# BesenbacherLab/kmerPaPa

Hardware: NVIDIA B200
Metric: pattern-scores/sec (higher is better)
Workload: dtype f64

## Files before the change

### kmerpapa_b200/csrc/kp_api.cu

```cuda
#include <cuda_runtime.h>
#include <math.h>
#include <stdio.h>
#include <stdlib.h>
#include <string.h>

#include <algorithm>
#include <string>
#include <vector>

#include "../../include/kmerpapa_b200.h"
#include "kp_kernels.cuh"
#include "kp_fiber.cuh"
#include "kp_plan.h"
#include "kp_shard_owners.h"

namespace {

thread_local std::string g_err;

int fail(const std::string &msg)
{
    g_err = msg;
    return KP_ERR;
}

int fail_capacity(const std::string &msg)
{
    g_err = msg;
    return KP_ERR_CAPACITY;
}

#define KP_CUDA(call)                                                                         \
    do {                                                                                      \
        cudaError_t e_ = (call);                                                              \
        if (e_ != cudaSuccess)                                                                \
            return fail(std::string(#call) + ": " + cudaGetErrorString(e_) + " (" + __FILE__ + ":" + \
                        std::to_string(__LINE__) + ")");                                      \
    } while (0)

}

#ifndef KP_PF_TOP
#define KP_PF_TOP 0
#endif
#ifndef KP_EVICT_TOP
#define KP_EVICT_TOP 0
#endif

struct kp_plan {
    KpHostPlan host;
    int device = 0;
    int sm_count = 0;
    KpTables *d_tab = nullptr;
    uint8_t *d_rowtab = nullptr;
    uint32_t *d_tiles = nullptr;
    uint8_t *d_genmask = nullptr;
    int *d_err = nullptr;
    uint32_t *d_counters = nullptr;
    uint8_t *d_tile_wave = nullptr;
    uint8_t *d_tile_done = nullptr;
    unsigned char *d_scratch = nullptr;
    size_t scratch_cap = 0;
    uint64_t launches = 0;
    int nwarps[2] = {0, 0};
    size_t smem_optin = 0;
    bool coop_launch = false;
    KpFiberTables *d_ftab = nullptr;
    uint8_t *d_fiberblob = nullptr;
    uint32_t *d_fibers = nullptr;
    size_t fiber_smem[2] = {0, 0};
    int fiber_dbg = 0;
    bool use_fiber = false;
    int pf_dist = KP_PF_DIST;
    int evict_top = KP_EVICT_TOP;
    bool coop_tail = true;
    int pf_bulk = 0;
    int pf_top = KP_PF_TOP;
    bool one_launch = false;
};

#define KP_RP_NN 232
#ifndef KP_FIBER_DEFAULT
#define KP_FIBER_DEFAULT false
#endif

template <bool WIDE>
static const void *dp_kernel_for_radix(int r0, int rp)
{
    switch (r0) {
    case 1: return (const void *)kp_dp_rows_kernel<1, WIDE, 0, 0>;
    case 3: return (const void *)kp_dp_rows_kernel<3, WIDE, 0, 0>;
    case 7: return (const void *)kp_dp_rows_kernel<7, WIDE, 0, 0>;
    default:
        return rp == KP_RP_NN ? (const void *)kp_dp_rows_kernel<15, WIDE, KP_RP_NN, 0>
                              : (const void *)kp_dp_rows_kernel<15, WIDE, 0, 0>;
    }
}

template <int R0, int RP, int SHARD>
static void launch_dp_r0(bool wide, int grid, int threads, size_t smem, cudaStream_t st, const KpDpParams &prm)
{
    if (wide) kp_dp_rows_kernel<R0, true, RP, SHARD><<<grid, threads, smem, st>>>(prm);
    else kp_dp_rows_kernel<R0, false, RP, SHARD><<<grid, threads, smem, st>>>(prm);
}

template <bool WIDE, int SHARD>
static const void *dp_kernel_sharded(int rp)
{
    return rp == KP_RP_NN ? (const void *)kp_dp_rows_kernel<15, WIDE, KP_RP_NN, SHARD>
                          : (const void *)kp_dp_rows_kernel<15, WIDE, 0, SHARD>;
}

static KpView single_view(const kp_plan *p, const float *best, const uint16_t *flags);

static float tree_sum(const unsigned long long *keys, const float *vals, size_t lo, size_t hi, int depth)
{
    if (hi - lo == 1) return vals[lo];
    const unsigned long long bit = 1ULL << (63 - depth);
    size_t a = lo, b = hi;
    while (a < b) {
        size_t mid = (a + b) / 2;
        if (keys[mid] & bit) b = mid; else a = mid + 1;
    }
    if (a == lo || a == hi) return tree_sum(keys, vals, lo, hi, depth + 1);
    volatile float l = tree_sum(keys, vals, lo, a, depth + 1), r = tree_sum(keys, vals, a, hi, depth + 1);
    volatile float sum = l + r;
    return sum;
}

static KpView single_view(const kp_plan *p, const float *best, const uint16_t *flags)
{
    KpView v;
    memset(&v, 0, sizeof v);
    v.best[0] = best;
    v.flags[0] = flags;
    v.hw_top = (uint32_t)p->host.t.ntiles;
    return v;
}

extern "C" {

const char *kp_last_error(void) { return g_err.c_str(); }
int kp_version(void) { return 100; }

static const void *dp_kernel_ptr(int r0, int rp, bool wide)
{
    return wide ? dp_kernel_for_radix<true>(r0, rp) : dp_kernel_for_radix<false>(r0, rp);
}

static int plan_create(const char *gen_pat, int device, bool lattice, kp_plan **out);

int kp_plan_create(const char *gen_pat, int device, kp_plan **out) { return plan_create(gen_pat, device, true, out); }

int kp_plan_create_lite(const char *gen_pat, int device, kp_plan **out) { return plan_create(gen_pat, device, false, out); }

static int plan_create(const char *gen_pat, int device, bool lattice, kp_plan **out)
{
    if (!gen_pat || !out) return fail("kp_plan_create: null argument");
    int ndev = 0;
    cudaError_t e = cudaGetDeviceCount(&ndev);
    if (e != cudaSuccess || ndev == 0)
        return fail(std::string("kp_plan_create: no CUDA device (") + cudaGetErrorString(e) + "); there is no CPU path");
    if (device < 0 || device >= ndev) return fail("kp_plan_create: bad device ordinal");
    KP_CUDA(cudaSetDevice(device));
    kp_plan *p = new kp_plan();
    std::string err;
    if (kp_build_host_plan(gen_pat, p->host, err, lattice)) { delete p; return fail("kp_plan_create: " + err); }
    p->device = device;
    cudaDeviceProp prop;
    KP_CUDA(cudaGetDeviceProperties(&prop, device));
    p->sm_count = prop.multiProcessorCount;
    const KpTables &t = p->host.t;
    KP_CUDA(cudaMalloc(&p->d_tab, sizeof(KpTables)));
    KP_CUDA(cudaMemcpy(p->d_tab, &t, sizeof(KpTables), cudaMemcpyHostToDevice));
    KP_CUDA(cudaMalloc(&p->d_rowtab, p->host.rowtab.size()));
    KP_CUDA(cudaMemcpy(p->d_rowtab, p->host.rowtab.data(), p->host.rowtab.size(), cudaMemcpyHostToDevice));
    KP_CUDA(cudaMalloc(&p->d_tiles, sizeof(uint32_t) * (p->host.tile_order.size() + 1)));
    KP_CUDA(cudaMemcpy(p->d_tiles, p->host.tile_order.data(), sizeof(uint32_t) * p->host.tile_order.size(), cudaMemcpyHostToDevice));
    KP_CUDA(cudaMalloc(&p->d_genmask, KP_MAXK));
    KP_CUDA(cudaMemcpy(p->d_genmask, p->host.gen_mask, KP_MAXK, cudaMemcpyHostToDevice));
    KP_CUDA(cudaMalloc(&p->d_err, sizeof(int)));
    KP_CUDA(cudaMemset(p->d_err, 0, sizeof(int)));
    KP_CUDA(cudaMalloc(&p->d_counters, sizeof(uint32_t) * 128));
    if (t.r0 == 15 && t.nhigh > 0 && lattice) {
        std::vector<uint8_t> tw(p->host.tile_order.size());
        for (size_t l = 0; l + 1 < p->host.hl_off.size(); l++)
            for (uint64_t i = p->host.hl_off[l]; i < p->host.hl_off[l + 1]; i++) tw[i] = (uint8_t)l;
        KP_CUDA(cudaMalloc(&p->d_tile_wave, tw.size()));
        KP_CUDA(cudaMemcpy(p->d_tile_wave, tw.data(), tw.size(), cudaMemcpyHostToDevice));
        KP_CUDA(cudaMalloc(&p->d_tile_done, tw.size()));
    }
    p->smem_optin = prop.sharedMemPerBlockOptin;
    if (p->host.ft.ok) {
        const KpFiberTables &f = p->host.ft;
        KP_CUDA(cudaMalloc(&p->d_ftab, sizeof(KpFiberTables)));
        KP_CUDA(cudaMemcpy(p->d_ftab, &f, sizeof(KpFiberTables), cudaMemcpyHostToDevice));
        KP_CUDA(cudaMalloc(&p->d_fiberblob, p->host.fibertab.size()));
        KP_CUDA(cudaMemcpy(p->d_fiberblob, p->host.fibertab.data(), p->host.fibertab.size(), cudaMemcpyHostToDevice));
        KP_CUDA(cudaMalloc(&p->d_fibers, sizeof(uint32_t) * (p->host.fiber_order.size() + 1)));
        KP_CUDA(cudaMemcpy(p->d_fibers, p->host.fiber_order.data(), sizeof(uint32_t) * p->host.fiber_order.size(), cudaMemcpyHostToDevice));
        for (int wide = 0; wide < 2; wide++) {
            const size_t need = kp_fiber_smem(f.ft_bytes, f.maxhs, t.tile_kmers, wide != 0).total;
            p->fiber_smem[wide] = need <= p->smem_optin ? need : 0;
        }
        KP_CUDA(cudaFuncSetAttribute((const void *)kp_dp_fiber_kernel<false>, cudaFuncAttributeMaxDynamicSharedMemorySize, (int)prop.sharedMemPerBlockOptin));
        KP_CUDA(cudaFuncSetAttribute((const void *)kp_dp_fiber_kernel<true>, cudaFuncAttributeMaxDynamicSharedMemorySize, (int)prop.sharedMemPerBlockOptin));
        p->use_fiber = KP_FIBER_DEFAULT;
        if (const char *e = getenv("KP_DP_KERNEL")) p->use_fiber = strcmp(e, "fiber") == 0;
        if (const char *e = getenv("KP_FIBER_DBG")) p->fiber_dbg = atoi(e);
    }
    p->coop_launch = prop.cooperativeLaunch != 0 && !getenv("KP_NO_COOP_BACKTRACK");
    if (const char *e = getenv("KP_PF_DIST")) p->pf_dist = atoi(e);
    if (const char *e = getenv("KP_EVICT_TOP")) p->evict_top = atoi(e);
    if (const char *e = getenv("KP_PF_TOP")) p->pf_top = atoi(e);
    if (const char *e = getenv("KP_PF_BULK")) p->pf_bulk = atoi(e);
    if (getenv("KP_NO_COOP_TAIL")) p->coop_tail = false;
    if (const char *e = getenv("KP_ONE_LAUNCH")) p->one_launch = e[0] == '1';
    for (int wide = 0; wide < 2; wide++) {
        size_t fixed = 2048 + t.rt_bytes, per_warp = t.warp_smem_bytes[wide];
        int nw = fixed < p->smem_optin ? (int)((p->smem_optin - fixed) / per_warp) : 0;
        if (nw > KP_MAX_WARPS) nw = KP_MAX_WARPS;
        p->nwarps[wide] = nw;
        KP_CUDA(cudaFuncSetAttribute(dp_kernel_ptr(t.r0, t.rp, wide), cudaFuncAttributeMaxDynamicSharedMemorySize,
                                     (int)prop.sharedMemPerBlockOptin));
        if (t.r0 == 15)
            KP_CUDA(cudaFuncSetAttribute(wide ? dp_kernel_sharded<true, 3>(t.rp) : dp_kernel_sharded<false, 3>(t.rp),
                                         cudaFuncAttributeMaxDynamicSharedMemorySize, (int)prop.sharedMemPerBlockOptin));
    }
    *out = p;
    return 0;
}

int kp_plan_destroy(kp_plan *p)
{
    if (!p) return 0;
    cudaSetDevice(p->device);
    cudaFree(p->d_tab);
    cudaFree(p->d_rowtab);
    cudaFree(p->d_tiles);
    cudaFree(p->d_genmask);
    cudaFree(p->d_err);
    cudaFree(p->d_counters);
    cudaFree(p->d_tile_wave);
    cudaFree(p->d_tile_done);
    cudaFree(p->d_ftab);
    cudaFree(p->d_fiberblob);
    cudaFree(p->d_fibers);
    cudaFree(p->d_scratch);
    delete p;
    return 0;
}

uint64_t kp_backtrack_ws_bytes(uint64_t cap) { return (3 * cap) * sizeof(KpBtNode) + cap * (8 + 8 + 4) + 80 * 8 + 64; }

int kp_plan_get_info(const kp_plan *p, kp_plan_info *o)
{
    if (!p || !o) return fail("kp_plan_get_info: null argument");
    const KpTables &t = p->host.t;
    memset(o, 0, sizeof *o);
    o->npat = p->host.npat;
    o->nkmer = p->host.nkmer;
    o->ntiles = t.ntiles;
    o->table_elems = (uint64_t)t.ntiles * t.tile_stride;
    o->kept_elems = (uint64_t)t.ntiles * (uint64_t)t.rp;
    o->expanded_elems = (uint64_t)t.ntiles * t.tile_kmers;
    o->backtrack_ws_bytes = kp_backtrack_ws_bytes(65536);
    o->k = (uint32_t)p->host.k;
    o->nlevels = t.total_level + 1;
    o->tile_cells = t.tile_cells;
    o->tile_stride = t.tile_stride;
    o->tile_kmers = t.tile_kmers;
    o->low_positions = (uint32_t)t.nlow;
    o->register_radix = (uint32_t)t.r0;
    o->rows = (uint32_t)t.nrows;
    o->rounds = (uint32_t)t.nrounds;
    o->warps_per_cta = (uint32_t)p->nwarps[0];
    o->high_levels = (uint32_t)(p->host.hl_off.size() - 1);
    o->sm_count = (uint32_t)p->sm_count;
    return 0;
}

uint64_t kp_plan_launch_count(const kp_plan *p) { return p ? p->launches : 0; }

const char *kp_dp_kernel_name(const kp_plan *p)
{
    return p && p->use_fiber && p->fiber_smem[0] ? "kp_dp_fiber_kernel" : "kp_dp_rows_kernel";
}

int kp_pattern_offset(const kp_plan *p, uint64_t patnum, uint64_t *table_elem, uint64_t *kept_elem, uint32_t *kept_bit)
{
    if (p && !p->host.lattice) return fail("kp_pattern_offset: this plan was created without the tile lattice (kp_plan_create_lite)");
    if (!p) return fail("kp_pattern_offset: null plan");
    if (patnum >= p->host.npat) return fail("kp_pattern_offset: pattern number out of range");
    uint64_t tile; uint32_t srow, d0;
    kp_locate(p->host, patnum, &tile, &srow, &d0);
    const KpTables &t = p->host.t;
    if (table_elem) *table_elem = tile * t.tile_stride + ((uint64_t)(d0 >> 2) * t.rp + srow) * 4 + (d0 & 3);
    if (kept_elem) *kept_elem = tile * (uint64_t)t.rp + srow;
    if (kept_bit) *kept_bit = d0;
    return 0;
}

static int scratch_reserve(kp_plan *p, size_t bytes, cudaStream_t st)
{
    if (bytes <= p->scratch_cap) return 0;
    KP_CUDA(cudaStreamSynchronize(st));
    if (p->d_scratch) KP_CUDA(cudaFree(p->d_scratch));
    p->d_scratch = nullptr;
    p->scratch_cap = 0;
    size_t cap = bytes + bytes / 2 + 4096;
    KP_CUDA(cudaMalloc(&p->d_scratch, cap));
    p->scratch_cap = cap;
    return 0;
}

static int grid_for(uint64_t n, int threads, int sm_count)
{
    uint64_t b = (n + threads - 1) / threads;
    uint64_t cap = (uint64_t)sm_count * 16;
    if (b > cap) b = cap;
    if (b < 1) b = 1;
    return (int)b;
}

int kp_pack_counts(kp_plan *p, const uint64_t *h_codes, const int64_t *h_pos, const int64_t *h_neg, uint64_t n,
                   int64_t *d_kmerM, int64_t *d_kmerU, void *stream)
{
    if (!p) return fail("kp_pack_counts: null plan");
    if (p->host.k > 16) return fail("kp_pack_counts: packed codes hold at most 16 positions");
    cudaStream_t st = (cudaStream_t)stream;
    KP_CUDA(cudaSetDevice(p->device));
    KP_CUDA(cudaMemsetAsync(d_kmerM, 0, p->host.nkmer * 8, st));
    KP_CUDA(cudaMemsetAsync(d_kmerU, 0, p->host.nkmer * 8, st));
    if (n == 0) return 0;
    if (scratch_reserve(p, n * 24, st)) return 1;
    unsigned long long *d_codes = (unsigned long long *)p->d_scratch;
    long long *d_pos = (long long *)(d_codes + n), *d_neg = d_pos + n;
    KP_CUDA(cudaMemcpyAsync(d_codes, h_codes, n * 8, cudaMemcpyHostToDevice, st));
    KP_CUDA(cudaMemcpyAsync(d_pos, h_pos, n * 8, cudaMemcpyHostToDevice, st));
    KP_CUDA(cudaMemcpyAsync(d_neg, h_neg, n * 8, cudaMemcpyHostToDevice, st));
    KP_CUDA(cudaMemsetAsync(p->d_err, 0, sizeof(int), st));
    kp_pack_kernel<<<grid_for(n, 256, p->sm_count), 256, 0, st>>>(p->d_tab, p->d_genmask, p->host.k, d_codes, d_pos, d_neg, n,
                                                                  (long long *)d_kmerM, (long long *)d_kmerU, p->d_err);
    p->launches++;
    KP_CUDA(cudaGetLastError());
    int herr = 0;
    KP_CUDA(cudaMemcpyAsync(&herr, p->d_err, sizeof(int), cudaMemcpyDeviceToHost, st));
    KP_CUDA(cudaStreamSynchronize(st));
    if (herr) return fail("kp_pack_counts: a k-mer code is not one-hot or lies outside the general pattern");
    return 0;
}

int kp_expand_counts(kp_plan *p, const int64_t *d_kmerM, const int64_t *d_kmerU, int64_t *d_expM, int64_t *d_expU,
                     void *stream)
{
    if (!p) return fail("kp_expand_counts: null plan");
    if (!p->host.lattice) return fail("kp_expand_counts: this plan was created without the tile lattice (kp_plan_create_lite)");
    cudaStream_t st = (cudaStream_t)stream;
    KP_CUDA(cudaSetDevice(p->device));
    const KpTables &t = p->host.t;
    kp_expand_base_kernel<<<grid_for(p->host.nkmer, 256, p->sm_count), 256, 0, st>>>(
        p->d_tab, p->host.nkmer, (const long long *)d_kmerM, (const long long *)d_kmerU, (long long *)d_expM, (long long *)d_expU);
    p->launches++;
    for (int hi = 0; hi < t.nhigh; hi++) {
        uint64_t total = t.tile_kmers;
        for (int h = 0; h < t.nhigh; h++) {
            const int f = t.highpos[h];
            total *= h < hi ? (uint64_t)t.radix[f] : (h == hi ? (uint64_t)(t.radix[f] - t.nbase[f]) : (uint64_t)t.nbase[f]);
        }
        if (total == 0) continue;
        kp_expand_pass_kernel<<<grid_for(total, 256, p->sm_count), 256, 0, st>>>(p->d_tab, hi, total, (long long *)d_expM,
                                                                                 (long long *)d_expU);
        p->launches++;
    }
    KP_CUDA(cudaGetLastError());
    return 0;
}

static int launch_dp(kp_plan *p, bool wide, KpDpParams prm, cudaStream_t st)
{
    if (!p->host.lattice) return fail("this plan was created without the tile lattice (kp_plan_create_lite): no DP");
    int nw = p->nwarps[wide];
    if (nw < 1) return fail("DP kernel does not fit in shared memory for this tile shape");
    size_t nhl = p->host.hl_off.size() - 1;
    const KpTables &t = p->host.t;
    if (nhl > 64) return fail("too many tile waves");
    KP_CUDA(cudaMemsetAsync(p->d_counters, 0, sizeof(uint32_t) * 128, st));
    if (p->use_fiber && p->fiber_smem[wide]) {
        KpFiberParams fp;
        memset(&fp, 0, sizeof fp);
        fp.tab = p->d_tab; fp.ftab = p->d_ftab; fp.fiberblob = p->d_fiberblob;
        fp.e0 = prm.e0; fp.e1 = prm.e1; fp.s0 = prm.s0; fp.s1 = prm.s1;
        fp.alpha = prm.alpha; fp.beta = prm.beta; fp.penalty = prm.penalty;
        fp.best = prm.best; fp.flags = prm.flags;
        fp.dbg = p->fiber_dbg;
        const size_t nfl = p->host.fl_off.size() - 1;
        for (size_t l = 0; l < nfl; l++) {
            const uint64_t lo = p->host.fl_off[l], hi = p->host.fl_off[l + 1];
            if (hi == lo) continue;
            fp.fiber_list = p->d_fibers + lo;
            fp.nfibers_wave = (uint32_t)(hi - lo);
            fp.counter = p->d_counters + l;
            fp.leaf_wave = (l == 0);
            const int grid = (int)std::min<uint64_t>(hi - lo, (uint64_t)p->sm_count);
            if (wide) kp_dp_fiber_kernel<true><<<grid, KP_FIBER_THREADS, p->fiber_smem[1], st>>>(fp);
            else kp_dp_fiber_kernel<false><<<grid, KP_FIBER_THREADS, p->fiber_smem[0], st>>>(fp);
            p->launches++;
        }
        KP_CUDA(cudaGetLastError());
        return 0;
    }
    if (p->d_tile_done && t.ntiles >= (uint64_t)8 * p->sm_count * nw && p->one_launch) {
        KP_CUDA(cudaMemsetAsync(p->d_tile_done, 0, t.ntiles, st));
        KP_CUDA(cudaMemsetAsync(p->d_err, 0, sizeof(int), st));
        prm.tile_list = p->d_tiles;
        prm.ntiles_wave = (uint32_t)t.ntiles;
        prm.counter = p->d_counters;
        prm.leaf_wave = 0;
        prm.tile_wave = p->d_tile_wave;
        prm.tile_done = p->d_tile_done;
        prm.wave_done = p->d_counters + 64;
        prm.err = p->d_err;
        for (size_t l = 0; l < 64; l++) prm.wave_size[l] = l < nhl ? (uint32_t)(p->host.hl_off[l + 1] - p->host.hl_off[l]) : 0;
        const size_t sm = 2048 + t.rt_bytes + (size_t)nw * t.warp_smem_bytes[wide];
        if (t.rp == KP_RP_NN) launch_dp_r0<15, KP_RP_NN, 3>(wide, p->sm_count, nw * 32, sm, st, prm);
        else launch_dp_r0<15, 0, 3>(wide, p->sm_count, nw * 32, sm, st, prm);
        p->launches++;
        KP_CUDA(cudaGetLastError());
        return 0;
    }
    for (size_t l = 0; l < nhl; l++) {
        uint64_t lo = p->host.hl_off[l], hi = p->host.hl_off[l + 1];
        if (hi == lo) continue;
        prm.tile_list = p->d_tiles + lo;
        prm.ntiles_wave = (uint32_t)(hi - lo);
        prm.counter = p->d_counters + l;
        prm.leaf_wave = (l == 0);
        uint64_t ntile = hi - lo;
        const int nchunk = (t.nrows + 31) / 32;
        if (p->coop_tail && t.r0 == 15 && ntile <= (uint64_t)p->sm_count && nchunk <= KP_MAX_WARPS) {
            const size_t smc = 2048 + t.rt_bytes + (size_t)t.warp_smem_bytes[wide];
            if (t.rp == KP_RP_NN) launch_dp_r0<15, KP_RP_NN, 4>(wide, (int)ntile, nchunk * 32, smc, st, prm);
            else launch_dp_r0<15, 0, 4>(wide, (int)ntile, nchunk * 32, smc, st, prm);
            p->launches++;
            continue;
        }
        int warps = nw;
        if (ntile < (uint64_t)p->sm_count * nw) {
            warps = (int)((ntile + p->sm_count - 1) / p->sm_count);
            if (warps < 1) warps = 1;
        }
        uint64_t grid = (ntile + warps - 1) / warps;
        if (grid > (uint64_t)p->sm_count) grid = p->sm_count;
        size_t sm = 2048 + t.rt_bytes + (size_t)warps * t.warp_smem_bytes[wide];
        switch (t.r0) {
        case 1: launch_dp_r0<1, 0, 0>(wide, (int)grid, warps * 32, sm, st, prm); break;
        case 3: launch_dp_r0<3, 0, 0>(wide, (int)grid, warps * 32, sm, st, prm); break;
        case 7: launch_dp_r0<7, 0, 0>(wide, (int)grid, warps * 32, sm, st, prm); break;
        default:
            if (t.rp == KP_RP_NN) launch_dp_r0<15, KP_RP_NN, 0>(wide, (int)grid, warps * 32, sm, st, prm);
            else launch_dp_r0<15, 0, 0>(wide, (int)grid, warps * 32, sm, st, prm);
            break;
        }
        p->launches++;
    }
    KP_CUDA(cudaGetLastError());
    return 0;
}

static int dp_counts(kp_plan *p, const int64_t *d_expM, const int64_t *d_expU, const int64_t *d_subM, const int64_t *d_subU,
                     uint64_t max_count, double alpha, double beta, double penalty, float *d_best, uint16_t *d_kept, void *stream);

int kp_dp_single(kp_plan *p, const int64_t *d_expM, const int64_t *d_expU, uint64_t max_count, double alpha, double beta,
                 double penalty, float *d_best, uint16_t *d_kept, void *stream)
{
    return dp_counts(p, d_expM, d_expU, nullptr, nullptr, max_count, alpha, beta, penalty, d_best, d_kept, stream);
}

static int dp_counts(kp_plan *p, const int64_t *d_expM, const int64_t *d_expU, const int64_t *d_subM, const int64_t *d_subU,
                     uint64_t max_count, double alpha, double beta, double penalty, float *d_best, uint16_t *d_kept, void *stream)
{
    if (!p) return fail("kp_dp_single: null plan");
    KP_CUDA(cudaSetDevice(p->device));
    bool wide = max_count > 0xFFFFFFFFull;
    KpDpParams prm;
    memset(&prm, 0, sizeof prm);
    prm.tab = p->d_tab;
    prm.rowtab = p->d_rowtab;
    prm.e0 = (const long long *)d_expM;
    prm.e1 = (const long long *)d_expU;
    prm.s0 = (const long long *)d_subM;
    prm.s1 = (const long long *)d_subU;
    prm.alpha = alpha; prm.beta = beta; prm.penalty = penalty;
    prm.best = d_best;
    prm.flags = d_kept;
    prm.pf_dist = p->pf_dist;
    prm.evict_top = p->evict_top < p->host.t.nhigh ? p->evict_top : 0;
    prm.pf_top = p->pf_top;
    prm.pf_bulk = p->pf_bulk;
    return launch_dp(p, wide, prm, (cudaStream_t)stream);
}

static int backtrack_device(kp_plan *p, const KpView &vw, void *d_ws, uint64_t cap, uint64_t root,
                            cudaStream_t st, unsigned long long **sorted_out, unsigned long long **keys_out, float **vals_out,
                            unsigned long long **ctr_out)
{
    KpBtNode *fa = (KpBtNode *)d_ws, *fb = fa + cap, *leaves = fb + cap;
    unsigned long long *sorted = (unsigned long long *)(leaves + cap);
    unsigned long long *keys = sorted + cap;
    unsigned long long *ctr = keys + cap;
    float *vals = (float *)(ctr + 80);
    kp_backtrack_init_kernel<<<1, 128, 0, st>>>(fa, root, ctr);
    const int levels = (int)p->host.t.total_level + 1;
    int grid = (int)((cap + 7) / 8);
    if (grid > p->sm_count * 2) grid = p->sm_count * 2;
    bool fused = false;
    if (p->coop_launch) {
        int nlev = levels < 64 ? levels : 64;
        int cgrid = grid < p->sm_count ? grid : p->sm_count;
        const KpTables *a_tab = p->d_tab;
        const uint8_t *a_row = p->d_rowtab;
        void *args[] = {(void *)&a_tab, (void *)&a_row, (void *)&vw, (void *)&nlev, (void *)&fa, (void *)&fb, (void *)&leaves,
                        (void *)&cap, (void *)&ctr};
        if (cudaLaunchCooperativeKernel((const void *)kp_backtrack_all_kernel, dim3(cgrid), dim3(256), args, 0, st) == cudaSuccess) {
            fused = true;
            p->launches++;
        } else {
            cudaGetLastError();
        }
    }
    for (int d = 0; !fused && d < levels && d < 64; d++) {
        kp_backtrack_level_kernel<<<grid, 256, 0, st>>>(p->d_tab, p->d_rowtab, vw, d, (d & 1) ? fb : fa,
                                                        (d & 1) ? fa : fb, leaves, cap, ctr);
        p->launches++;
    }
    kp_backtrack_sort_kernel<<<p->sm_count, 256, 0, st>>>(leaves, ctr, cap, sorted, keys);
    p->launches += 2;
    KP_CUDA(cudaGetLastError());
    *sorted_out = sorted; *keys_out = keys; *vals_out = vals; *ctr_out = ctr;
    return 0;
}

int kp_backtrack(kp_plan *p, const float *d_best, const uint16_t *d_kept, void *d_ws, uint64_t cap, uint64_t root,
                 uint64_t *h_patnums, uint64_t *n_out, void *stream)
{
    if (!p || !d_ws || !h_patnums || !n_out) return fail("kp_backtrack: null argument");
    if (p->host.t.total_level > 64) return fail("kp_backtrack: more than 64 levels");
    if (root == UINT64_MAX) root = p->host.npat - 1;
    if (root >= p->host.npat) return fail("kp_backtrack: root out of range");
    cudaStream_t st = (cudaStream_t)stream;
    KP_CUDA(cudaSetDevice(p->device));
    unsigned long long *sorted, *keys, *ctr;
    float *vals;
    if (backtrack_device(p, single_view(p, d_best, d_kept), d_ws, cap, root, st, &sorted, &keys, &vals, &ctr)) return 1;
    unsigned long long hc[2] = {0, 0};
    int herr = 0;
    KP_CUDA(cudaMemcpyAsync(hc, ctr, sizeof hc, cudaMemcpyDeviceToHost, st));
    KP_CUDA(cudaMemcpyAsync(&herr, p->d_err, sizeof herr, cudaMemcpyDeviceToHost, st));
    KP_CUDA(cudaStreamSynchronize(st));
    if (herr == 2) return fail("kp_backtrack: the DP gave up waiting for a child tile (internal error)");
    *n_out = hc[0];
    if (hc[1] || hc[0] > cap) return fail_capacity("kp_backtrack: partition larger than the workspace capacity");
    KP_CUDA(cudaMemcpyAsync(h_patnums, sorted, hc[0] * 8, cudaMemcpyDeviceToHost, st));
    KP_CUDA(cudaStreamSynchronize(st));
    return 0;
}

int kp_cv_heldout(kp_plan *p, const float *d_train, const uint16_t *d_kept, const int64_t *d_expMtot, const int64_t *d_expUtot,
                  const int64_t *d_expMtest, const int64_t *d_expUtest, double alpha, double beta_fold, double penalty,
                  uint64_t root, void *d_ws, uint64_t cap, float *h_test, void *stream)
{
    if (!p || !d_ws || !h_test) return fail("kp_cv_heldout: null argument");
    if (root == UINT64_MAX) root = p->host.npat - 1;
    if (root >= p->host.npat) return fail("kp_cv_heldout: root out of range");
    cudaStream_t st = (cudaStream_t)stream;
    KP_CUDA(cudaSetDevice(p->device));
    unsigned long long *sorted, *keys, *ctr;
    float *vals;
    if (backtrack_device(p, single_view(p, d_train, d_kept), d_ws, cap, root, st, &sorted, &keys, &vals, &ctr)) return 1;
    kp_cv_leaf_kernel<<<p->sm_count, 128, 0, st>>>(p->d_tab, p->d_rowtab, (const long long *)d_expMtot, (const long long *)d_expUtot,
                                                   (const long long *)d_expMtest, (const long long *)d_expUtest, alpha, beta_fold,
                                                   penalty, sorted, ctr, cap, vals);
    p->launches++;
    KP_CUDA(cudaGetLastError());
    unsigned long long hc[2] = {0, 0};
    KP_CUDA(cudaMemcpyAsync(hc, ctr, sizeof hc, cudaMemcpyDeviceToHost, st));
    KP_CUDA(cudaStreamSynchronize(st));
    if (hc[1] || hc[0] > cap) return fail_capacity("kp_cv_heldout: partition larger than the workspace capacity");
    if (hc[0] == 0) return fail("kp_cv_heldout: the backtrack produced no leaf (internal error)");
    std::vector<unsigned long long> hk(hc[0]);
    std::vector<float> hv(hc[0]);
    KP_CUDA(cudaMemcpyAsync(hk.data(), keys, hc[0] * 8, cudaMemcpyDeviceToHost, st));
    KP_CUDA(cudaMemcpyAsync(hv.data(), vals, hc[0] * 4, cudaMemcpyDeviceToHost, st));
    KP_CUDA(cudaStreamSynchronize(st));
    *h_test = tree_sum(hk.data(), hv.data(), 0, hc[0], 0);
    return 0;
}

int kp_dp_cv_job(kp_plan *p, const int64_t *d_expMtot, const int64_t *d_expUtot, const int64_t *d_expMtest,
                 const int64_t *d_expUtest, uint64_t max_count, double alpha, double beta_fold, double penalty,
                 float *d_train, uint16_t *d_kept, void *d_ws, uint64_t cap, float *h_top, void *stream)
{
    if (!p || !d_expMtest || !d_expUtest) return fail("kp_dp_cv_job: null argument");
    cudaStream_t st = (cudaStream_t)stream;
    KP_CUDA(cudaSetDevice(p->device));
    const KpTables &t = p->host.t;
    if (dp_counts(p, d_expMtot, d_expUtot, d_expMtest, d_expUtest, max_count, alpha, beta_fold, penalty, d_train, d_kept, stream))
        return 1;
    if (h_top) {
        if (int rc = kp_cv_heldout(p, d_train, d_kept, d_expMtot, d_expUtot, d_expMtest, d_expUtest, alpha, beta_fold, penalty,
                                   UINT64_MAX, d_ws, cap, h_top + 1, stream))
            return rc;
        uint64_t tile; uint32_t srow, d0;
        kp_locate(p->host, p->host.npat - 1, &tile, &srow, &d0);
        size_t top = (size_t)tile * t.tile_stride + ((size_t)(d0 >> 2) * t.rp + srow) * 4 + (d0 & 3);
        KP_CUDA(cudaMemcpyAsync(h_top, d_train + top, sizeof(float), cudaMemcpyDeviceToHost, st));
        KP_CUDA(cudaStreamSynchronize(st));
    }
    return 0;
}

uint64_t kp_cv_stage_bytes(uint64_t cap) { return 32 + cap * 12; }

int kp_cv_job_enqueue(kp_plan *p, const int64_t *d_expMtot, const int64_t *d_expUtot, const int64_t *d_expMtest,
                      const int64_t *d_expUtest, uint64_t max_count, double alpha, double beta_fold, double penalty,
                      float *d_train, uint16_t *d_kept, void *d_ws, uint64_t cap, void *h_stage, void *stream)
{
    if (!p || !d_expMtest || !d_expUtest || !d_ws || !h_stage) return fail("kp_cv_job_enqueue: null argument");
    cudaStream_t st = (cudaStream_t)stream;
    KP_CUDA(cudaSetDevice(p->device));
    const KpTables &t = p->host.t;
    if (dp_counts(p, d_expMtot, d_expUtot, d_expMtest, d_expUtest, max_count, alpha, beta_fold, penalty, d_train, d_kept, stream))
        return 1;
    unsigned long long *sorted, *keys, *ctr;
    float *vals;
    if (backtrack_device(p, single_view(p, d_train, d_kept), d_ws, cap, p->host.npat - 1, st, &sorted, &keys, &vals, &ctr)) return 1;
    kp_cv_leaf_kernel<<<p->sm_count, 128, 0, st>>>(p->d_tab, p->d_rowtab, (const long long *)d_expMtot, (const long long *)d_expUtot,
                                                   (const long long *)d_expMtest, (const long long *)d_expUtest, alpha, beta_fold,
                                                   penalty, sorted, ctr, cap, vals);
    p->launches++;
    KP_CUDA(cudaGetLastError());
    unsigned char *h = (unsigned char *)h_stage;
    uint64_t tile; uint32_t srow, d0;
    kp_locate(p->host, p->host.npat - 1, &tile, &srow, &d0);
    const size_t top = (size_t)tile * t.tile_stride + ((size_t)(d0 >> 2) * t.rp + srow) * 4 + (d0 & 3);
    KP_CUDA(cudaMemcpyAsync(h, ctr, 16, cudaMemcpyDeviceToHost, st));
    KP_CUDA(cudaMemcpyAsync(h + 16, d_train + top, sizeof(float), cudaMemcpyDeviceToHost, st));
    KP_CUDA(cudaMemcpyAsync(h + 32, keys, cap * 8, cudaMemcpyDeviceToHost, st));
    KP_CUDA(cudaMemcpyAsync(h + 32 + cap * 8, vals, cap * 4, cudaMemcpyDeviceToHost, st));
    return 0;
}

int kp_cv_job_finish(const void *h_stage, uint64_t cap, float *h_top)
{
    if (!h_stage || !h_top) return fail("kp_cv_job_finish: null argument");
    const unsigned char *h = (const unsigned char *)h_stage;
    unsigned long long hc[2];
    memcpy(hc, h, 16);
    if (hc[1] || hc[0] > cap) return fail_capacity("kp_cv_job_finish: partition larger than the workspace capacity");
    if (hc[0] == 0) return fail("kp_cv_job_finish: the backtrack produced no leaf (internal error)");
    memcpy(h_top, h + 16, sizeof(float));
    h_top[1] = tree_sum((const unsigned long long *)(h + 32), (const float *)(h + 32 + cap * 8), 0, hc[0], 0);
    return 0;
}

int kp_split_codes(kp_plan *p, const float *d_best, const uint16_t *d_kept, const uint64_t *h_patnums, uint64_t n,
                   uint8_t *h_codes, void *stream)
{
    if (!p) return fail("kp_split_codes: null plan");
    if (n == 0) return 0;
    cudaStream_t st = (cudaStream_t)stream;
    KP_CUDA(cudaSetDevice(p->device));
    if (scratch_reserve(p, n * 9, st)) return 1;
    unsigned long long *d_pat = (unsigned long long *)p->d_scratch;
    uint8_t *d_codes = (uint8_t *)(d_pat + n);
    KP_CUDA(cudaMemcpyAsync(d_pat, h_patnums, n * 8, cudaMemcpyHostToDevice, st));
    kp_split_codes_kernel<<<grid_for(n, 256, p->sm_count), 256, 0, st>>>(p->d_tab, p->d_rowtab, single_view(p, d_best, d_kept), d_pat, n, d_codes);
    p->launches++;
    KP_CUDA(cudaGetLastError());
    KP_CUDA(cudaMemcpyAsync(h_codes, d_codes, n, cudaMemcpyDeviceToHost, st));
    KP_CUDA(cudaStreamSynchronize(st));
    return 0;
}

int kp_gather_table(kp_plan *p, const float *d_table, uint64_t first, uint64_t n, float *h_out, void *stream)
{
    if (!p) return fail("kp_gather_table: null plan");
    if (n == 0) return 0;
    cudaStream_t st = (cudaStream_t)stream;
    KP_CUDA(cudaSetDevice(p->device));
    if (scratch_reserve(p, n * 4, st)) return 1;
    float *d_out = (float *)p->d_scratch;
    kp_gather_kernel<<<grid_for(n, 256, p->sm_count), 256, 0, st>>>(p->d_tab, p->d_rowtab, single_view(p, d_table, nullptr), nullptr, first, n, d_out);
    p->launches++;
    KP_CUDA(cudaGetLastError());
    KP_CUDA(cudaMemcpyAsync(h_out, d_out, n * 4, cudaMemcpyDeviceToHost, st));
    KP_CUDA(cudaStreamSynchronize(st));
    return 0;
}

int kp_gather_kept(kp_plan *p, const uint16_t *d_kept, uint64_t first, uint64_t n, uint8_t *h_out, void *stream)
{
    if (!p) return fail("kp_gather_kept: null plan");
    if (n == 0) return 0;
    cudaStream_t st = (cudaStream_t)stream;
    KP_CUDA(cudaSetDevice(p->device));
    if (scratch_reserve(p, n, st)) return 1;
    uint8_t *d_out = (uint8_t *)p->d_scratch;
    kp_gather_flags_kernel<<<grid_for(n, 256, p->sm_count), 256, 0, st>>>(p->d_tab, p->d_rowtab, single_view(p, nullptr, d_kept), nullptr, first, n, d_out);
    p->launches++;
    KP_CUDA(cudaGetLastError());
    KP_CUDA(cudaMemcpyAsync(h_out, d_out, n, cudaMemcpyDeviceToHost, st));
    KP_CUDA(cudaStreamSynchronize(st));
    return 0;
}

int kp_gather_patterns(kp_plan *p, const float *d_table, const uint16_t *d_kept, const uint64_t *h_patnums, uint64_t n,
                       float *h_best, uint8_t *h_kept, uint8_t *h_codes, void *stream)
{
    if (!p || !h_patnums) return fail("kp_gather_patterns: null argument");
    if (!p->host.lattice) return fail("kp_gather_patterns: this plan was created without the tile lattice (kp_plan_create_lite)");
    if ((h_best || h_codes) && !d_table) return fail("kp_gather_patterns: scores and split codes need the score table");
    if ((h_kept || h_codes) && !d_kept) return fail("kp_gather_patterns: kept flags and split codes need the kept-whole table");
    if (n == 0) return 0;
    cudaStream_t st = (cudaStream_t)stream;
    KP_CUDA(cudaSetDevice(p->device));
    if (scratch_reserve(p, n * 16, st)) return 1;
    unsigned long long *d_pat = (unsigned long long *)p->d_scratch;
    float *d_val = (float *)(d_pat + n);
    uint8_t *d_k = (uint8_t *)(d_val + n), *d_c = d_k + n;
    KP_CUDA(cudaMemcpyAsync(d_pat, h_patnums, n * 8, cudaMemcpyHostToDevice, st));
    const int grid = grid_for(n, 256, p->sm_count);
    const KpView vw = single_view(p, d_table, d_kept);
    if (h_best) { kp_gather_kernel<<<grid, 256, 0, st>>>(p->d_tab, p->d_rowtab, vw, d_pat, 0, n, d_val); p->launches++; }
    if (h_kept) { kp_gather_flags_kernel<<<grid, 256, 0, st>>>(p->d_tab, p->d_rowtab, vw, d_pat, 0, n, d_k); p->launches++; }
    if (h_codes) { kp_split_codes_kernel<<<grid, 256, 0, st>>>(p->d_tab, p->d_rowtab, vw, d_pat, n, d_c); p->launches++; }
    KP_CUDA(cudaGetLastError());
    if (h_best) KP_CUDA(cudaMemcpyAsync(h_best, d_val, n * 4, cudaMemcpyDeviceToHost, st));
    if (h_kept) KP_CUDA(cudaMemcpyAsync(h_kept, d_k, n, cudaMemcpyDeviceToHost, st));
    if (h_codes) KP_CUDA(cudaMemcpyAsync(h_codes, d_c, n, cudaMemcpyDeviceToHost, st));
    KP_CUDA(cudaStreamSynchronize(st));
    return 0;
}

int kp_pattern_counts(kp_plan *p, const int64_t *d_kmerM, const int64_t *d_kmerU, const uint64_t *h_patnums, uint64_t n,
                      int64_t *h_M, int64_t *h_U, void *stream)
{
    if (!p) return fail("kp_pattern_counts: null plan");
    if (n == 0) return 0;
    cudaStream_t st = (cudaStream_t)stream;
    KP_CUDA(cudaSetDevice(p->device));
    if (scratch_reserve(p, n * 24, st)) return 1;
    unsigned long long *d_pat = (unsigned long long *)p->d_scratch;
    long long *d_out = (long long *)(d_pat + n);
    KP_CUDA(cudaMemcpyAsync(d_pat, h_patnums, n * 8, cudaMemcpyHostToDevice, st));
    const int pc_grid = (int)std::min<uint64_t>(n, (uint64_t)p->sm_count * 16);
    kp_pattern_counts_kernel<<<pc_grid, 256, 0, st>>>(p->d_tab, n, (const long long *)d_kmerM, (const long long *)d_kmerU,
                                                      d_pat, d_out, d_out + n);
    p->launches++;
    KP_CUDA(cudaGetLastError());
    KP_CUDA(cudaMemcpyAsync(h_M, d_out, n * 8, cudaMemcpyDeviceToHost, st));
    KP_CUDA(cudaMemcpyAsync(h_U, d_out + n, n * 8, cudaMemcpyDeviceToHost, st));
    KP_CUDA(cudaStreamSynchronize(st));
    return 0;
}

struct PartLayout {
    unsigned long long *pat, *pm, *offs, *bsum;
};

static size_t part_bytes(uint64_t n) { return (3 * n + 1 + 1024) * 8; }

static PartLayout part_layout(const kp_plan *p, uint64_t n)
{
    PartLayout L;
    L.pat = (unsigned long long *)p->d_scratch;
    L.pm = L.pat + n;
    L.offs = L.pm + n;
    L.bsum = L.offs + n + 1;
    return L;
}

static int part_check(const kp_plan *p, const char *what, const uint64_t *h_patnums, uint64_t n)
{
    if (!p) return fail(std::string(what) + ": null plan");
    if (!h_patnums || n == 0) return fail(std::string(what) + ": empty partition");
    if (n >= KP_OWNER_EMPTY) return fail(std::string(what) + ": too many patterns (owners are uint32)");
    for (uint64_t i = 0; i < n; i++)
        if (h_patnums[i] >= p->host.npat) return fail(std::string(what) + ": pattern number out of range");
    return 0;
}

static int part_prepare(kp_plan *p, const uint64_t *h_patnums, uint64_t n, cudaStream_t st, uint64_t *total)
{
    const PartLayout L = part_layout(p, n);
    KP_CUDA(cudaMemcpyAsync(L.pat, h_patnums, n * 8, cudaMemcpyHostToDevice, st));
    const uint64_t nb = std::min<uint64_t>(1024, (n + 255) / 256), per = (n + nb - 1) / nb;
    kp_part_prep_kernel<<<(unsigned)nb, 256, 0, st>>>(p->d_tab, L.pat, n, per, L.pm, L.bsum);
    kp_part_scan_kernel<<<1, 256, 0, st>>>(L.bsum, (unsigned)nb, L.offs, n);
    kp_part_offsets_kernel<<<(unsigned)nb, 256, 0, st>>>(p->d_tab, L.pm, n, per, L.bsum, L.offs);
    p->launches += 3;
    KP_CUDA(cudaGetLastError());
    unsigned long long tot = 0;
    KP_CUDA(cudaMemcpyAsync(&tot, L.offs + n, 8, cudaMemcpyDeviceToHost, st));
    KP_CUDA(cudaStreamSynchronize(st));
    *total = tot;
    return 0;
}

int kp_partition_assign(kp_plan *p, const uint64_t *h_patnums, uint64_t n, uint32_t *d_owner, uint64_t *h_conflict,
                        uint64_t *h_uncovered, void *stream)
{
    if (part_check(p, "kp_partition_assign", h_patnums, n)) return KP_ERR;
    if (!d_owner || !h_conflict || !h_uncovered) return fail("kp_partition_assign: null argument");
    cudaStream_t st = (cudaStream_t)stream;
    KP_CUDA(cudaSetDevice(p->device));
    if (scratch_reserve(p, part_bytes(n) + 16, st)) return KP_ERR;
    const PartLayout L = part_layout(p, n);
    unsigned long long *d_res = L.bsum + 1024;
    uint64_t total = 0;
    if (part_prepare(p, h_patnums, n, st, &total)) return KP_ERR;
    const uint64_t nkmer = p->host.nkmer;
    KP_CUDA(cudaMemsetAsync(d_owner, 0xFF, nkmer * 4, st));
    KP_CUDA(cudaMemsetAsync(d_res, 0xFF, 16, st));
    const int grid = p->sm_count * 8;
    unsigned long long res[2] = {~0ull, ~0ull};
    for (uint64_t lo = 0; lo < total; lo += nkmer) {
        const uint64_t hi = std::min<uint64_t>(total, lo + nkmer);
        kp_part_assign_kernel<<<grid, 256, 0, st>>>(p->d_tab, L.pm, L.offs, n, lo, hi, d_owner, d_res);
        p->launches++;
        KP_CUDA(cudaGetLastError());
        if (hi == total) break;
        KP_CUDA(cudaMemcpyAsync(res, d_res, 8, cudaMemcpyDeviceToHost, st));
        KP_CUDA(cudaStreamSynchronize(st));
        if (res[0] != ~0ull) break;
    }
    KP_CUDA(cudaMemcpyAsync(res, d_res, 8, cudaMemcpyDeviceToHost, st));
    KP_CUDA(cudaStreamSynchronize(st));
    if (res[0] == ~0ull) {
        kp_part_cover_kernel<<<grid_for(nkmer, 256, p->sm_count), 256, 0, st>>>(d_owner, nkmer, d_res);
        p->launches++;
        KP_CUDA(cudaGetLastError());
        KP_CUDA(cudaMemcpyAsync(res, d_res, 16, cudaMemcpyDeviceToHost, st));
        KP_CUDA(cudaStreamSynchronize(st));
    }
    *h_conflict = res[0] == ~0ull ? 0 : res[0] + 1;
    *h_uncovered = res[0] != ~0ull || res[1] == ~0ull ? 0 : res[1] + 1;
    return 0;
}

int kp_partition_score(kp_plan *p, const uint64_t *h_patnums, const double *h_rate, uint64_t n, const int64_t *d_kmerM,
                       const int64_t *d_kmerU, const uint32_t *d_owner, double *d_kmer_rate, int64_t *h_M, int64_t *h_U,
                       double *h_t, void *stream)
{
    if (part_check(p, "kp_partition_score", h_patnums, n)) return KP_ERR;
    if (!h_rate || !d_kmerM || !d_kmerU || !h_M || !h_U || !h_t) return fail("kp_partition_score: null argument");
    if (d_kmer_rate && !d_owner) return fail("kp_partition_score: the per-k-mer rates need the owner table");
    cudaStream_t st = (cudaStream_t)stream;
    KP_CUDA(cudaSetDevice(p->device));
    if (scratch_reserve(p, part_bytes(n) + 4 * n * 8, st)) return KP_ERR;
    const PartLayout L = part_layout(p, n);
    unsigned long long *d_M = (unsigned long long *)((unsigned char *)p->d_scratch + part_bytes(n)), *d_U = d_M + n;
    double *d_rate = (double *)(d_U + n), *d_t = d_rate + n;
    uint64_t total = 0;
    if (part_prepare(p, h_patnums, n, st, &total)) return KP_ERR;
    if (total > p->host.nkmer) return fail("kp_partition_score: the patterns have more members than there are k-mers (they overlap)");
    KP_CUDA(cudaMemcpyAsync(d_rate, h_rate, n * 8, cudaMemcpyHostToDevice, st));
    KP_CUDA(cudaMemsetAsync(d_M, 0, 2 * n * 8, st));
    kp_part_counts_kernel<<<p->sm_count * 8, 256, 0, st>>>(p->d_tab, L.pm, L.offs, n, total, (const long long *)d_kmerM,
                                                           (const long long *)d_kmerU, d_M, d_U);
    kp_part_terms_kernel<<<grid_for(n, 256, p->sm_count), 256, 0, st>>>(d_M, d_U, d_rate, n, d_t);
    p->launches += 2;
    if (d_kmer_rate) {
        kp_part_kmer_rate_kernel<<<grid_for(p->host.nkmer, 256, p->sm_count), 256, 0, st>>>(d_owner, d_rate, n, p->host.nkmer,
                                                                                           d_kmer_rate);
        p->launches++;
    }
    KP_CUDA(cudaGetLastError());
    KP_CUDA(cudaMemcpyAsync(h_M, d_M, n * 8, cudaMemcpyDeviceToHost, st));
    KP_CUDA(cudaMemcpyAsync(h_U, d_U, n * 8, cudaMemcpyDeviceToHost, st));
    KP_CUDA(cudaMemcpyAsync(h_t, d_t, n * 8, cudaMemcpyDeviceToHost, st));
    KP_CUDA(cudaStreamSynchronize(st));
    return 0;
}

int kp_kmer_rates(kp_plan *p, const uint32_t *d_owner, const double *h_rate, uint64_t n, double *d_kmer_rate, void *stream)
{
    if (!p) return fail("kp_kmer_rates: null plan");
    if (!d_owner || !h_rate || !d_kmer_rate || n == 0) return fail("kp_kmer_rates: null argument");
    cudaStream_t st = (cudaStream_t)stream;
    KP_CUDA(cudaSetDevice(p->device));
    if (scratch_reserve(p, n * 8, st)) return KP_ERR;
    double *d_rate = (double *)p->d_scratch;
    KP_CUDA(cudaMemcpyAsync(d_rate, h_rate, n * 8, cudaMemcpyHostToDevice, st));
    kp_part_kmer_rate_kernel<<<grid_for(p->host.nkmer, 256, p->sm_count), 256, 0, st>>>(d_owner, d_rate, n, p->host.nkmer,
                                                                                       d_kmer_rate);
    p->launches++;
    KP_CUDA(cudaGetLastError());
    KP_CUDA(cudaStreamSynchronize(st));
    return 0;
}

int kp_seq_scan(kp_plan *p, const uint8_t *d_seq, uint64_t seq_base, uint64_t seq_len, uint64_t rec_len, uint64_t pos0,
                uint64_t pos1, int both, const double *d_kmer_rate, const uint32_t *d_tasks, uint64_t ntask, double *d_sum,
                int64_t *d_n, float *d_track, const uint32_t *d_count_mask, int64_t *d_counts, void *stream)
{
    if (!p) return fail("kp_seq_scan: null plan");
    const int k = p->host.k, c = k / 2;
    if (!d_seq || !d_kmer_rate || !d_sum || !d_n) return fail("kp_seq_scan: null argument");
    if ((uintptr_t)d_seq & 15) return fail("kp_seq_scan: the sequence buffer must be 16-byte aligned");
    if (both && k % 2 == 0) return fail("kp_seq_scan: both strands need an odd k");
    if (pos0 % KP_SEQ_PIECE || pos0 > pos1 || pos1 > rec_len) return fail("kp_seq_scan: bad position range");
    const uint64_t need_lo = pos0 >= (uint64_t)c ? pos0 - c : 0, need_hi = std::min<uint64_t>(rec_len, pos1 + (k - 1 - c));
    if (pos1 > pos0 && (seq_base > need_lo || seq_base + seq_len < need_hi || seq_base + seq_len > rec_len))
        return fail("kp_seq_scan: the sequence bytes do not cover the windows of the positions");
    if (d_tasks && (d_track || d_counts)) return fail("kp_seq_scan: tracks and counts come from the whole-piece pass");
    if (pos1 == pos0 || (d_tasks && ntask == 0)) return 0;
    if (!d_tasks && (pos1 - pos0 + KP_SEQ_PIECE - 1) / KP_SEQ_PIECE > 0x7FFFFFFFull) return fail("kp_seq_scan: too many pieces");
    if (d_tasks && ntask > 0x7FFFFFFFull) return fail("kp_seq_scan: too many tasks");
    cudaStream_t st = (cudaStream_t)stream;
    KP_CUDA(cudaSetDevice(p->device));
    KpSeqScan a;
    a.seq = d_seq;
    a.seq_base = seq_base;
    a.seq_len = seq_len;
    a.rec_len = rec_len;
    a.pos0 = pos0;
    a.pos1 = pos1;
    a.kmer_rate = d_kmer_rate;
    a.tasks = d_tasks;
    a.sum = d_sum;
    a.n = (unsigned long long *)d_n;
    a.track = d_track;
    a.count_mask = d_count_mask;
    a.counts = (unsigned long long *)d_counts;
    a.k = k;
    a.c = c;
    const unsigned grid = (unsigned)(d_tasks ? ntask : (pos1 - pos0 + KP_SEQ_PIECE - 1) / KP_SEQ_PIECE);
    if (both) kp_seq_scan_kernel<true><<<grid, KP_SEQ_THREADS, 0, st>>>(p->d_tab, p->d_genmask, a);
    else kp_seq_scan_kernel<false><<<grid, KP_SEQ_THREADS, 0, st>>>(p->d_tab, p->d_genmask, a);
    p->launches++;
    KP_CUDA(cudaGetLastError());
    return 0;
}

int kp_region_sums(kp_plan *p, const double *d_piece_sum, const int64_t *d_piece_n, const double *d_task_sum,
                   const int64_t *d_task_n, const int64_t *d_regions, uint64_t n, double *d_sum, int64_t *d_n, void *stream)
{
// ... 659 lines not shown
```

### kmerpapa_b200/csrc/kp_fiber.cuh

```cuda
#pragma once
#include "kp_kernels.cuh"

#define KP_FIBER_THREADS 512
#define KP_FIBER_CELLS (KP_FIBER_DIGITS * KP_FIBER_ROWS)

struct KpFiberParams {
    const KpTables *tab;
    const KpFiberTables *ftab;
    const uint8_t *fiberblob;
    const uint32_t *fiber_list;
    uint32_t nfibers_wave;
    uint32_t *counter;
    int leaf_wave;
    const long long *e0, *e1;
    const long long *s0, *s1;
    double alpha, beta, penalty;
    float *best;
    uint16_t *flags;
    int dbg;
};

struct KpFiberSmem {
    uint32_t logtab, blob, bc, hs, misc, fsplit, flags, planes, total;
};

__host__ __device__ inline KpFiberSmem kp_fiber_smem(uint32_t ft_bytes, uint32_t maxhs, uint32_t tile_kmers, bool wide)
{
    KpFiberSmem m;
    uint32_t o = 0;
    m.logtab = o; o += 2048;
    m.blob = o; o += (ft_bytes + 15u) & ~15u;
    m.bc = o; o += KP_FIBER_DIGITS * tile_kmers * 2u * (wide ? 8u : 4u);
    m.hs = o; o += ((maxhs * 8u) + 15u) & ~15u;
    m.misc = o; o += 256;
    m.fsplit = o; o += 256;
    m.flags = o; o += (KP_FIBER_CELLS * 2u + 15u) & ~15u;
    m.planes = o; o += KP_FIBER_CELLS * 60u;
    m.total = o;
    return m;
}

struct KpFiberS {
    float4 *P0, *P1, *P2;
    float *Q0, *Q1, *Q2;
    __device__ __forceinline__ void load(int idx, float *v) const
    {
        const float4 a = P0[idx], b = P1[idx], c = P2[idx];
        v[0] = a.x; v[1] = a.y; v[2] = a.z; v[3] = a.w;
        v[4] = b.x; v[5] = b.y; v[6] = b.z; v[7] = b.w;
        v[8] = c.x; v[9] = c.y; v[10] = c.z; v[11] = c.w;
        v[12] = Q0[idx]; v[13] = Q1[idx]; v[14] = Q2[idx];
    }
    __device__ __forceinline__ void store(int idx, const float *v) const
    {
        P0[idx] = make_float4(v[0], v[1], v[2], v[3]);
        P1[idx] = make_float4(v[4], v[5], v[6], v[7]);
        P2[idx] = make_float4(v[8], v[9], v[10], v[11]);
        Q0[idx] = v[12]; Q1[idx] = v[13]; Q2[idx] = v[14];
    }
};

__device__ __forceinline__ void kp_fiber_split1(const KpFiberS &S, int ia, int ib, float *v)
{
    float xa[16], xb[16];
    S.load(ia, xa);
    S.load(ib, xb);
#pragma unroll
    for (int c = 0; c < 14; c += 2) {
        const float2 s = __fadd2_rn(make_float2(xa[c], xa[c + 1]), make_float2(xb[c], xb[c + 1]));
        v[c] = fminf(v[c], s.x);
        v[c + 1] = fminf(v[c + 1], s.y);
    }
    v[14] = fminf(v[14], __fadd_rn(xa[14], xb[14]));
}

__device__ __forceinline__ void kp_fiber_split2(const KpFiberS &S, int ia, int ib, int ic, int ie, float *v)
{
    float xa[16], xb[16], xc[16], xe[16];
    S.load(ia, xa);
    S.load(ib, xb);
    S.load(ic, xc);
    S.load(ie, xe);
#pragma unroll
    for (int c = 0; c < 14; c += 2) {
        const float2 s1 = __fadd2_rn(make_float2(xa[c], xa[c + 1]), make_float2(xb[c], xb[c + 1]));
        const float2 s2 = __fadd2_rn(make_float2(xc[c], xc[c + 1]), make_float2(xe[c], xe[c + 1]));
        v[c] = kp_min3(v[c], s1.x, s2.x);
        v[c + 1] = kp_min3(v[c + 1], s1.y, s2.y);
    }
    v[14] = kp_min3(v[14], __fadd_rn(xa[14], xb[14]), __fadd_rn(xc[14], xe[14]));
}

__device__ __forceinline__ float4 kp_min4(float4 m, float4 a, float4 b)
{
    const float2 lo = __fadd2_rn(make_float2(a.x, a.y), make_float2(b.x, b.y));
    const float2 hi = __fadd2_rn(make_float2(a.z, a.w), make_float2(b.z, b.w));
    return make_float4(fminf(m.x, lo.x), fminf(m.y, lo.y), fminf(m.z, hi.x), fminf(m.w, hi.y));
}

template <bool WIDE>
__global__ void __launch_bounds__(KP_FIBER_THREADS, 1) kp_dp_fiber_kernel(const KpFiberParams p)
{
    typedef typename KpCnt<WIDE>::type C;
    constexpr int R0 = 15, NB = 4, NT = KP_FIBER_THREADS, NR = KP_FIBER_ROWS, RP = 232;
    constexpr int TILE4 = 4 * RP;
    constexpr int NJ = KP_FIBER_DIGITS * TILE4;

    extern __shared__ __align__(16) unsigned char smem[];
    const KpTables &tb = *p.tab;
    const KpFiberTables &ft = *p.ftab;
    const int tid = threadIdx.x;
    const uint32_t tk = tb.tile_kmers;
    const KpFiberSmem sm = kp_fiber_smem(ft.ft_bytes, ft.maxhs, tk, WIDE);

    double2 *logtab = (double2 *)(smem + sm.logtab);
    unsigned char *blob = smem + sm.blob;
    C *bc = (C *)(smem + sm.bc);
    uint32_t *hs1 = (uint32_t *)(smem + sm.hs), *hs2 = hs1 + ft.maxhs;
    int *misc = (int *)(smem + sm.misc);
    uint8_t *fsplit = smem + sm.fsplit;
    uint16_t *sflags = (uint16_t *)(smem + sm.flags);
    KpFiberS S;
    S.P0 = (float4 *)(smem + sm.planes);
    S.P1 = S.P0 + KP_FIBER_CELLS;
    S.P2 = S.P1 + KP_FIBER_CELLS;
    S.Q0 = (float *)(S.P2 + KP_FIBER_CELLS);
    S.Q1 = S.Q0 + KP_FIBER_CELLS;
    S.Q2 = S.Q1 + KP_FIBER_CELLS;

    for (int i = tid; i < 128; i += NT) logtab[i] = make_double2(kpc_logTab[2 * i], kpc_logTab[2 * i + 1]);
    for (uint32_t i = tid; i < ft.ft_bytes / 4; i += NT) ((uint32_t *)blob)[i] = ((const uint32_t *)p.fiberblob)[i];
    if (tid < KP_FIBER_DIGITS) {
        const int e = ft.fe, d = tid;
        const uint32_t m = tb.digit_mask[e][d];
        const int ns = tb.ms_n[m];
        for (int j = 0; j < ns; j++) {
            fsplit[(d * 8 + j) * 2 + 0] = tb.mask_digit[e][tb.ms_c1[m][j]];
            fsplit[(d * 8 + j) * 2 + 1] = tb.mask_digit[e][tb.ms_c2[m][j]];
        }
        fsplit[240 + d] = (uint8_t)ns;
    }
    __syncthreads();
    const uint8_t *frow_of_srow = blob + ft.ft_frow_of_srow;
    const uint16_t *xs_off = (const uint16_t *)(blob + ft.ft_xs_off);
    const uint16_t *xs = (const uint16_t *)(blob + ft.ft_xs);
    const uint16_t *bs_off = (const uint16_t *)(blob + ft.ft_bs_off);
    const uint8_t *bs = blob + ft.ft_bs;
    uint32_t lvl_start[KP_FIBER_ROW_LEVELS + 1];
#pragma unroll
    for (int l = 0; l <= KP_FIBER_ROW_LEVELS; l++) lvl_start[l] = ft.lvl_start[l];

    const double alpha = p.alpha, beta = p.beta, penalty = p.penalty;
    const KpFilterK fk = kp_filter_consts(alpha, beta, penalty);
    const float INF = __int_as_float(0x7f800000);
    const uint32_t hwf = ft.hw;
    const int nhigh = tb.nhigh, fhi = ft.fhi;
    const float4 *tb4 = (const float4 *)p.best;

    for (;;) {
        __syncthreads();
        if (tid == 0) misc[0] = (int)atomicAdd(p.counter, 1u);
        __syncthreads();
        const uint32_t it = (uint32_t)misc[0];
        if (it >= p.nfibers_wave) break;
        const uint32_t base = p.fiber_list[it];
        if (tid < 32) {
            int ns = 0, d = 0, e = 0;
            uint32_t m = 0, hw = 1;
            if (tid < nhigh && tid != fhi) {
                e = tb.highpos[tid];
                hw = tb.highw[e];
                d = (int)((base / hw) % tb.radix[e]);
                m = tb.digit_mask[e][d];
                ns = tb.ms_n[m];
            }
            int off = ns;
#pragma unroll
            for (int o = 1; o < 32; o <<= 1) {
                int x = __shfl_up_sync(0xffffffffu, off, o);
                if (tid >= o) off += x;
            }
            const int total = __shfl_sync(0xffffffffu, off, 31);
            off -= ns;
            for (int j = 0; j < ns; j++) {
                const int c1 = tb.mask_digit[e][tb.ms_c1[m][j]], c2 = tb.mask_digit[e][tb.ms_c2[m][j]];
                hs1[off + j] = base - (uint32_t)(d - c1) * hw;
                hs2[off + j] = base - (uint32_t)(d - c2) * hw;
            }
            if (tid == 0) misc[1] = total;
        }
        for (uint32_t i = tid; i < KP_FIBER_DIGITS * tk; i += NT) {
            const uint32_t x = i / tk, kl = i - x * tk;
            const size_t g = (size_t)(base + x * hwf) * tk + kl;
            bc[i * 2 + 0] = (C)(p.s0 ? p.e0[g] - p.s0[g] : p.e0[g]);
            bc[i * 2 + 1] = (C)(p.s1 ? p.e1[g] - p.s1[g] : p.e1[g]);
        }
        __syncthreads();
        const int nhs = misc[1];

        for (int j0 = tid; j0 < ((p.dbg & 1) ? 0 : NJ); j0 += 2 * NT) {
            const int j1 = j0 + NT;
            const int x0 = j0 / TILE4, r0 = j0 - x0 * TILE4;
            const int x1 = j1 / TILE4, r1 = j1 - x1 * TILE4;
            const int g0 = r0 / RP, srow0 = r0 - g0 * RP;
            const int g1 = r1 / RP, srow1 = r1 - g1 * RP;
            const bool ok0 = srow0 < NR, ok1 = j1 < NJ && srow1 < NR;
            const size_t o0 = (size_t)x0 * hwf * TILE4 + r0, o1 = (size_t)x1 * hwf * TILE4 + r1;
            float4 acc0 = make_float4(INF, INF, INF, INF), acc1 = acc0;
            for (int s0 = 0; s0 < nhs; s0 += 4) {
                float4 a0[4], b0[4], a1[4], b1[4];
#pragma unroll
                for (int q = 0; q < 4; q++) {
                    a0[q] = b0[q] = a1[q] = b1[q] = make_float4(INF, INF, INF, INF);
                    if (s0 + q < nhs) {
                        const float4 *c1 = tb4 + (size_t)hs1[s0 + q] * TILE4, *c2 = tb4 + (size_t)hs2[s0 + q] * TILE4;
                        if (ok0) { a0[q] = __ldg(c1 + o0); b0[q] = __ldg(c2 + o0); }
                        if (ok1) { a1[q] = __ldg(c1 + o1); b1[q] = __ldg(c2 + o1); }
                    }
                }
#pragma unroll
                for (int q = 0; q < 4; q++) {
                    acc0 = kp_min4(acc0, a0[q], b0[q]);
                    acc1 = kp_min4(acc1, a1[q], b1[q]);
                }
            }
            if (ok0) {
                const int idx = x0 * NR + frow_of_srow[srow0];
                if (g0 == 0) S.P0[idx] = acc0;
                else if (g0 == 1) S.P1[idx] = acc0;
                else if (g0 == 2) S.P2[idx] = acc0;
                else { S.Q0[idx] = acc0.x; S.Q1[idx] = acc0.y; S.Q2[idx] = acc0.z; }
            }
            if (ok1) {
                const int idx = x1 * NR + frow_of_srow[srow1];
                if (g1 == 0) S.P0[idx] = acc1;
                else if (g1 == 1) S.P1[idx] = acc1;
                else if (g1 == 2) S.P2[idx] = acc1;
                else { S.Q0[idx] = acc1.x; S.Q1[idx] = acc1.y; S.Q2[idx] = acc1.z; }
            }
        }
        __syncthreads();

        for (int L = 0; L <= ((p.dbg & 2) ? -1 : 3 + KP_FIBER_ROW_LEVELS - 1); L++) {
            int gstart[5];
            gstart[0] = 0;
#pragma unroll
            for (int lx = 0; lx < 4; lx++) {
                const int lr = L - lx;
                const int nx = lx == 0 ? 4 : (lx == 1 ? 6 : (lx == 2 ? 4 : 1));
                int nr = 0;
#pragma unroll
                for (int l = 0; l < KP_FIBER_ROW_LEVELS; l++)
                    if (l == lr) nr = (int)(lvl_start[l + 1] - lvl_start[l]);
                gstart[lx + 1] = gstart[lx] + nx * nr;
            }
            for (int k = tid; k < gstart[4]; k += NT) {
                const int lx = k < gstart[1] ? 0 : (k < gstart[2] ? 1 : (k < gstart[3] ? 2 : 3));
                const int lr = L - lx;
                const int xbase = lx == 0 ? 0 : (lx == 1 ? 4 : (lx == 2 ? 10 : 14));
                int rstart = 0, nr = 1;
#pragma unroll
                for (int l = 0; l < KP_FIBER_ROW_LEVELS; l++)
                    if (l == lr) { rstart = (int)lvl_start[l]; nr = (int)(lvl_start[l + 1] - lvl_start[l]); }
                const int kk = k - gstart[lx];
                const int xi = kk / nr;
                const int x = xbase + xi, frow = rstart + (kk - xi * nr);
                const int idx = x * NR + frow;

                float v[16];
                S.load(idx, v);
                v[15] = INF;
                {
                    const int nfs = fsplit[240 + x];
                    const uint8_t *fs = fsplit + x * 16;
                    int j = 0;
                    for (; j + 2 <= nfs; j += 2)
                        kp_fiber_split2(S, fs[2 * j] * NR + frow, fs[2 * j + 1] * NR + frow, fs[2 * j + 2] * NR + frow,
                                        fs[2 * j + 3] * NR + frow, v);
                    if (j < nfs) kp_fiber_split1(S, fs[2 * j] * NR + frow, fs[2 * j + 1] * NR + frow, v);
                }
                {
                    int i = xs_off[frow];
                    const int iend = xs_off[frow + 1];
                    const int xb = x * NR;
                    for (; i + 2 <= iend; i += 2) {
                        const uint32_t pr = xs[i], pq = xs[i + 1];
                        kp_fiber_split2(S, xb + (int)(pr & 0xFFu), xb + (int)(pr >> 8), xb + (int)(pq & 0xFFu), xb + (int)(pq >> 8), v);
                    }
                    if (i < iend) {
                        const uint32_t pr = xs[i];
                        kp_fiber_split1(S, xb + (int)(pr & 0xFFu), xb + (int)(pr >> 8), v);
                    }
                }
                C m[NB], u[NB];
#pragma unroll
                for (int b = 0; b < NB; b++) { m[b] = 0; u[b] = 0; }
                {
                    const C *bcx = bc + (size_t)x * tk * 2;
                    for (int i = bs_off[frow]; i < bs_off[frow + 1]; i++) {
                        const C *q = bcx + (size_t)bs[i] * NB * 2;
                        if (!WIDE) {
#pragma unroll
                            for (int b = 0; b < NB; b += 2) {
                                const uint4 y = *(const uint4 *)(q + b * 2);
                                m[b] += y.x; u[b] += y.y; m[b + 1] += y.z; u[b + 1] += y.w;
                            }
                        } else {
#pragma unroll
                            for (int b = 0; b < NB; b++) { m[b] += q[b * 2 + 0]; u[b] += q[b * 2 + 1]; }
                        }
                    }
                }
                const bool leafrow = p.leaf_wave != 0 && lx == 0 && lr == 0;
                uint32_t need = 0;
                {
                    float mf[NB], uf[NB];
#pragma unroll
                    for (int b = 0; b < NB; b++) { mf[b] = (float)m[b]; uf[b] = (float)u[b]; }
#pragma unroll
                    for (int h = 0; h < (R0 + 1) / 2; h++) {
                        float2 Mf = make_float2(0.f, 0.f), Uf = make_float2(0.f, 0.f);
#pragma unroll
                        for (int b = 0; b < NB; b++) {
                            if ((kp_bm_c<R0>(2 * h) >> b) & 1) { Mf.x += mf[b]; Uf.x += uf[b]; }
                            if (2 * h + 1 < R0 && ((kp_bm_c<R0>(2 * h + 1) >> b) & 1)) { Mf.y += mf[b]; Uf.y += uf[b]; }
                        }
                        const float2 lb = kp_score_lower_bound2(Mf, Uf, fk);
                        if (!(lb.x > v[2 * h])) need |= 1u << (2 * h);
                        if (2 * h + 1 < R0 && !(lb.y > v[2 * h + 1])) need |= 1u << (2 * h + 1);
                    }
                    if (leafrow) need |= (1u << NB) - 1u;
                }
                float sfx[16];
#pragma unroll
                for (int c = 0; c < 16; c++) sfx[c] = 0.f;
                uint32_t rupm = 0;
                if (need) {
                    const KpLogK K = kp_logk_load();
                    uint32_t todo = need;
                    while (todo) {
                        const int d = __ffs(todo) - 1;
                        todo &= todo - 1;
                        const unsigned bm = kp_bm<R0>(d);
                        C M_ = 0, U_ = 0;
#pragma unroll
                        for (int b = 0; b < NB; b++)
                            if ((bm >> b) & 1u) { M_ += m[b]; U_ += u[b]; }
                        float sf;
                        bool ru;
                        const bool leafcell = leafrow && d < NB;
                        if (leafcell || !kp_self_score_fast<C>(M_, U_, alpha, beta, penalty, logtab, K, sf, ru)) {
                            const double s_ = leafcell ? kp_leaf_score_nl(M_, U_, alpha, beta, penalty, logtab)
                                                       : kp_self_score_exact_nl<C>(M_, U_, alpha, beta, penalty, logtab);
                            sf = __double2float_rn(s_);
                            ru = (double)sf > s_;
                        }
                        if (ru) rupm |= 1u << d;
#pragma unroll
                        for (int c = 0; c < R0; c++)
                            if (c == d) sfx[c] = sf;
                    }
                }
                uint32_t flag = 0;
#define KP_FIN(D)                                                                                     \
    if ((need >> (D)) & 1u) {                                                                         \
        const float sf_ = sfx[D];                                                                     \
        if (sf_ < v[D] || (sf_ == v[D] && ((rupm >> (D)) & 1u))) { v[D] = sf_; flag |= 1u << (D); }   \
    }
#define KP_SP(D, A, B) v[D] = fminf(v[D], __fadd_rn(v[A], v[B]));
#define KP_SP2(D, A, B, A2, B2) v[D] = kp_min3(v[D], __fadd_rn(v[A], v[B]), __fadd_rn(v[A2], v[B2]));
                KP_FIN(0) KP_FIN(1) KP_FIN(2) KP_FIN(3)
                KP_SP(4, 0, 2) KP_FIN(4)
                KP_SP(5, 1, 3) KP_FIN(5)
                KP_SP(6, 2, 1) KP_FIN(6)
                KP_SP(7, 0, 3) KP_FIN(7)
                KP_SP(8, 2, 3) KP_FIN(8)
                KP_SP(9, 0, 1) KP_FIN(9)
                KP_SP2(10, 1, 8, 2, 5) KP_SP(10, 3, 6) KP_FIN(10)
                KP_SP2(11, 0, 8, 2, 7) KP_SP(11, 3, 4) KP_FIN(11)
                KP_SP2(12, 0, 5, 1, 7) KP_SP(12, 3, 9) KP_FIN(12)
                KP_SP2(13, 0, 6, 1, 4) KP_SP(13, 2, 9) KP_FIN(13)
                KP_SP2(14, 6, 7, 8, 9) KP_SP2(14, 4, 5, 0, 10)
                KP_SP2(14, 1, 11, 2, 12) KP_SP(14, 3, 13) KP_FIN(14)
#undef KP_FIN
#undef KP_SP
#undef KP_SP2
                S.store(idx, v);
                sflags[idx] = (uint16_t)flag;
            }
            __syncthreads();
        }

        for (int j = tid; j < NJ; j += NT) {
            const int x = j / TILE4, r = j - x * TILE4;
            const int g = r / RP, srow = r - g * RP;
            if (srow >= NR) continue;
            const int idx = x * NR + frow_of_srow[srow];
            float4 o;
            if (g == 0) o = S.P0[idx];
            else if (g == 1) o = S.P1[idx];
            else if (g == 2) o = S.P2[idx];
            else o = make_float4(S.Q0[idx], S.Q1[idx], S.Q2[idx], 0.f);
            __stcs((float4 *)p.best + (size_t)(base + x * hwf) * TILE4 + r, o);
        }
        for (int j = tid; j < KP_FIBER_DIGITS * RP; j += NT) {
            const int x = j / RP, srow = j - x * RP;
            if (srow < NR) p.flags[(size_t)(base + x * hwf) * RP + srow] = sflags[x * NR + frow_of_srow[srow]];
        }
    }
}
```

### kmerpapa_b200/csrc/kp_kernels.cuh

```cuda
#pragma once
#include <cuda_runtime.h>
#include <stdint.h>

#include "kp_math.cuh"
#include "kp_tables.h"

#ifndef KP_MAX_WARPS
#define KP_MAX_WARPS 12
#endif
#define KP_DP_BOUNDS __launch_bounds__(KP_MAX_WARPS * 32, 1)
#ifndef KP_PIPE_DEPTH
#define KP_PIPE_DEPTH 2
#endif
#ifndef KP_EXPERIMENTS
#define KP_EXPERIMENTS 0
#endif
#ifndef KP_PF_DIST
#define KP_PF_DIST 2
#endif

template <bool WIDE> struct KpCnt { typedef unsigned int type; };
template <> struct KpCnt<true> { typedef unsigned long long type; };

__device__ __forceinline__ double kp_cnt2d(unsigned int x) { return __uint2double_rn(x); }
__device__ __forceinline__ double kp_cnt2d(unsigned long long x) { return __ull2double_rn(x); }

template <typename C>
__device__ __forceinline__ double kp_self_score_t(C M, C U, double alpha, double beta, double penalty,
                                                  const double2 *tab, const KpLogK &K, double &logp, double &log1mp)
{
    double Md = kp_cnt2d(M), Ud = kp_cnt2d(U);
    double p = __ddiv_rn(KP_ADD(Md, alpha), KP_ADD(KP_ADD(kp_cnt2d((C)(M + U)), alpha), beta));
    double q = KP_SUB(1.0, p);
    int phi = __double2hiint(p), qhi = __double2hiint(q), qlo = __double2loint(q);
    if (kp_log_is_plain(phi) && !kp_log_is_near1(phi)) logp = kp_log_main(phi, __double2loint(p), tab, K);
    else logp = kp_log_slow(p, tab);
    if (kp_log_is_near1(qhi) && !(qhi == 0x3ff00000 && qlo == 0)) log1mp = kp_log_near1(q, K);
    else log1mp = kp_log_slow(q, tab);
    double s1 = KP_ADD(penalty, KP_MUL(KP_MUL(-2.0, Md), logp));
    double s = M > 0 ? s1 : penalty;
    double s2 = KP_ADD(s, KP_MUL(KP_MUL(-2.0, Ud), log1mp));
    return U > 0 ? s2 : s;
}

template <typename C>
__device__ __noinline__ double kp_self_score_exact_nl(C M, C U, double alpha, double beta, double penalty, const double2 *tab)
{
    const KpLogK K = kp_logk_load();
    double lp, l1;
    return kp_self_score_t<C>(M, U, alpha, beta, penalty, tab, K, lp, l1);
}

#ifndef KP_FAST_INLINE
#define KP_FAST_INLINE __forceinline__
#endif
template <typename C>
__device__ KP_FAST_INLINE bool kp_self_score_fast(C M, C U, double alpha, double beta, double penalty, const double2 *tab,
                                                   const KpLogK &K, float &sf, bool &rup, double *st = nullptr)
{
    const double Md = kp_cnt2d(M), Ud = kp_cnt2d(U), Sd = kp_cnt2d((C)(M + U));
    const double num = KP_ADD(Md, alpha), den = KP_ADD(KP_ADD(Sd, alpha), beta);
    double r;
    asm("rcp.approx.ftz.f64 %0, %1;" : "=d"(r) : "d"(den));
    double e = KP_FMA(-den, r, 1.0);
    r = KP_FMA(r, e, r);
    e = KP_FMA(-den, r, 1.0);
    r = KP_FMA(r, e, r);
    const double p = KP_MUL(num, r);
    const int phi = __double2hiint(p), dhi = __double2hiint(den);
    bool ok = (unsigned)(phi - 0x01700000) < (unsigned)(0x3fb00000 - 0x01700000) &&
              (unsigned)(dhi - 0x20b00000) < (unsigned)(0x5f300000 - 0x20b00000) && penalty >= 0.0;
    const double *A = kpc_logA;
    const unsigned thi = (unsigned)phi - 0x3fe60000u;
    const int i = (int)((thi >> 13) & 127u);
    const int k = (int)thi >> 20;
    const double z = __hiloint2double(phi - (int)(thi & 0xfff00000u), __double2loint(p));
    const double2 t = tab[i];
    const double kd = (double)k;
    const double rr = KP_FMA(z, t.x, -1.0);
    const double r2 = KP_MUL(rr, rr);
    const double w = KP_FMA(kd, KP_LOG_LN2HI, t.y);
    double q1 = KP_FMA(rr, A[4], K.a3);
    const double q5 = KP_FMA(rr, A[2], K.a1);
    q1 = KP_FMA(q1, r2, q5);
    double lo = KP_FMA(kd, KP_LOG_LN2LO, rr);
    lo = KP_FMA(r2, A[0], lo);
    lo = KP_FMA(KP_MUL(rr, r2), q1, lo);
    const double logp = KP_ADD(w, lo);
    const double *B = kpc_logB;
    const double x = KP_SUB(KP_SUB(1.0, p), 1.0);
    const double x2 = KP_MUL(x, x);
    double y;
    if (phi < 0x3f700000) {
        y = KP_FMA(x, B[4], B[3]);
        y = KP_FMA(y, x, B[2]);
        y = KP_FMA(y, x, K.b1);
        y = KP_FMA(y, x, -0.5);
    } else {
        y = KP_FMA(x, B[10], B[9]);
        y = KP_FMA(y, x, B[8]);
        y = KP_FMA(y, x, K.b7);
        y = KP_FMA(y, x, B[6]);
        y = KP_FMA(y, x, B[5]);
        y = KP_FMA(y, x, K.b4);
        y = KP_FMA(y, x, B[3]);
        y = KP_FMA(y, x, B[2]);
        y = KP_FMA(y, x, K.b1);
        y = KP_FMA(y, x, -0.5);
    }
    const double logq = KP_FMA(x2, y, x);
    const double t1 = KP_MUL(KP_MUL(-2.0, Md), logp), t2 = KP_MUL(KP_MUL(-2.0, Ud), logq);
    double sa = M > 0 ? KP_ADD(penalty, t1) : penalty;
    sa = U > 0 ? KP_ADD(sa, t2) : sa;
    const double eps = KP_FMA(sa, 0x1p-46, KP_MUL(Sd, 0x1p-49));
    const double slo = KP_SUB(sa, eps), shi = KP_ADD(sa, eps);
    const float flo = __double2float_rn(slo), fhi = __double2float_rn(shi);
    const double fd = (double)flo;
    sf = flo;
    rup = fd > shi;
    if (st) *st = sa;
    ok = ok && flo == fhi && (fd > shi || fd < slo) && sa < 0x1p120;
    return ok;
}

template <typename C>
__device__ __forceinline__ double kp_test_ll_t(C Mt, C Ut, double logp, double log1mp)
{
    double t1 = KP_ADD(0.0, KP_MUL(KP_MUL(-2.0, kp_cnt2d(Mt)), logp));
    double t = Mt > 0 ? t1 : 0.0;
    double t2 = KP_ADD(t, KP_MUL(KP_MUL(-2.0, kp_cnt2d(Ut)), log1mp));
    return Ut > 0 ? t2 : t;
}

template <int BM, int NB, typename C>
__device__ __forceinline__ C kp_sum_bases(const C *x)
{
    C s = 0;
#pragma unroll
    for (int b = 0; b < NB; b++)
        if ((BM >> b) & 1) s += x[b];
    return s;
}

template <int R0> __host__ __device__ constexpr int kp_bm_c(int d)
{
    return R0 == 15 ? (d == 0 ? 1 : d == 1 ? 2 : d == 2 ? 4 : d == 3 ? 8 : d == 4 ? 5 : d == 5 ? 10 : d == 6 ? 6 : d == 7 ? 9 :
                       d == 8 ? 12 : d == 9 ? 3 : d == 10 ? 14 : d == 11 ? 13 : d == 12 ? 11 : d == 13 ? 7 : d == 14 ? 15 : 0)
         : R0 == 7 ? (d == 0 ? 1 : d == 1 ? 2 : d == 2 ? 4 : d == 3 ? 3 : d == 4 ? 5 : d == 5 ? 6 : d == 6 ? 7 : 0)
         : R0 == 3 ? (d == 0 ? 1 : d == 1 ? 2 : d == 2 ? 3 : 0)
         : (d == 0 ? 1 : 0);
}

__device__ __noinline__ double kp_leaf_score_nl(unsigned long long M, unsigned long long U, double alpha, double beta,
                                                double penalty, const double2 *tab)
{
    return kp_leaf_score(M, U, alpha, beta, penalty, tab);
}
__device__ __noinline__ void kp_leaf_cv_nl(unsigned long long Mtr, unsigned long long Utr, unsigned long long Mte,
                                           unsigned long long Ute, double alpha, double beta, double penalty,
                                           const double2 *tab, double *train, double *test)
{
    double a, b;
    kp_leaf_cv(Mtr, Utr, Mte, Ute, alpha, beta, penalty, tab, a, b);
    *train = a;
    *test = b;
}

__constant__ uint8_t kpc_bm1[4] = {1, 0, 0, 0};
__constant__ uint8_t kpc_bm3[4] = {1, 2, 3, 0};
__constant__ uint8_t kpc_bm7[8] = {1, 2, 4, 3, 5, 6, 7, 0};
__constant__ uint8_t kpc_bm15[16] = {1, 2, 4, 8, 5, 10, 6, 9, 12, 3, 14, 13, 11, 7, 15, 0};
template <int R0> __device__ __forceinline__ unsigned kp_bm(int d)
{
    return R0 == 15 ? kpc_bm15[d] : (R0 == 7 ? kpc_bm7[d] : (R0 == 3 ? kpc_bm3[d] : kpc_bm1[d]));
}

__device__ __forceinline__ float kp_min3(float a, float b, float c)
{
    float r;
    asm("min.f32 %0, %1, %2, %3;" : "=f"(r) : "f"(a), "f"(b), "f"(c));
    return r;
}

struct KpFilterK { float alpha, ab, penalty, base; };
__device__ __forceinline__ KpFilterK kp_filter_consts(double alpha, double beta, double penalty)
{
    KpFilterK f;
    f.alpha = (float)alpha;
    f.ab = (float)(alpha + beta);
    f.penalty = (float)penalty;
    f.base = penalty >= 0.0 ? 0.01f : __fmaf_rn(4e-4f, (float)-penalty, 0.01f);
    return f;
}

__device__ __forceinline__ float2 kp_score_lower_bound2(float2 Mf, float2 Uf, const KpFilterK &f)
{
    const float2 num = __fadd2_rn(Mf, make_float2(f.alpha, f.alpha));
    const float2 cnt = __fadd2_rn(Mf, Uf);
    const float2 den = __fadd2_rn(cnt, make_float2(f.ab, f.ab));
    const float2 p = make_float2(__fdividef(num.x, den.x), __fdividef(num.y, den.y));
    const float2 lp = make_float2(__logf(p.x), __logf(p.y));
    float2 t = __ffma2_rn(p, make_float2(0.25f, 0.25f), make_float2(0.33333334f, 0.33333334f));
    t = __ffma2_rn(p, t, make_float2(0.5f, 0.5f));
    t = __ffma2_rn(p, t, make_float2(1.0f, 1.0f));
    float2 l1 = __fmul2_rn(make_float2(-p.x, -p.y), t);
    float2 rel = make_float2(1e-5f, 1e-5f), per = make_float2(0x1p-52f, 0x1p-52f);
    if (!(p.x < 0.03125f)) { l1.x = __logf(1.0f - p.x); rel.x = 2e-4f; per.x = 4e-6f; }
    if (!(p.y < 0.03125f)) { l1.y = __logf(1.0f - p.y); rel.y = 2e-4f; per.y = 4e-6f; }
    const float2 ll = __ffma2_rn(Mf, lp, __fmul2_rn(Uf, l1));
    const float2 est = __ffma2_rn(ll, make_float2(-2.0f, -2.0f), make_float2(f.penalty, f.penalty));
    const float2 mar = __ffma2_rn(make_float2(fabsf(est.x), fabsf(est.y)), rel, __ffma2_rn(cnt, per, make_float2(f.base, f.base)));
    return __fadd2_rn(est, make_float2(-mar.x, -mar.y));
}

__device__ __forceinline__ float4 kp_ldg_policy(const float4 *ptr, unsigned long long policy)
{
    float4 v;
    asm("ld.global.nc.L2::cache_hint.v4.f32 {%0, %1, %2, %3}, [%4], %5;"
        : "=f"(v.x), "=f"(v.y), "=f"(v.z), "=f"(v.w) : "l"(ptr), "l"(policy));
    return v;
}

#define KP_MAX_SHARDS 8
struct KpView {
    const float *best[KP_MAX_SHARDS];
    const uint16_t *flags[KP_MAX_SHARDS];
    uint32_t hw_top;
    uint8_t owner[16], slot[16];
    uint8_t push_mask[16];
    uint32_t hw_second;
    uint32_t two_d;
    uint8_t owner2[256];
    uint8_t push_mask2[256];
};

__device__ __forceinline__ void kp_view_tile(const KpView &v, unsigned long long tile, int &rank, unsigned long long &ltile)
{
    if (v.two_d) {
        rank = v.owner2[tile / v.hw_second];
        ltile = tile;
        return;
    }
    const unsigned long long d = tile / v.hw_top;
    rank = v.owner[d];
    ltile = (unsigned long long)v.slot[d] * v.hw_top + (tile - d * v.hw_top);
}

struct KpDpParams {
    const KpTables *tab;
    const uint8_t *rowtab;
    const uint32_t *tile_list;
    uint32_t ntiles_wave;
    uint32_t *counter;
    int leaf_wave;
    int pf_dist;
    int evict_top;
    int pf_top;
    int pf_bulk;
    const long long *e0, *e1;
    const long long *s0, *s1;
    double alpha, beta, penalty;
    float *best;
    uint16_t *flags;
    KpView view;
    int my_rank;
    const uint8_t *tile_wave;
    uint8_t *tile_done;
    uint32_t *wave_done;
    uint32_t wave_size[64];
    int *err;
};

template <int R0, bool WIDE, int RP, int SHARD>
__global__ void KP_DP_BOUNDS kp_dp_rows_kernel(const KpDpParams p)
{
    typedef typename KpCnt<WIDE>::type C;
    constexpr int NG = (R0 + 3) / 4;
    constexpr int NB = R0 == 15 ? 4 : (R0 == 7 ? 3 : (R0 == 3 ? 2 : 1));
    constexpr bool SHARDED = SHARD == 1;
    constexpr bool ONE_LAUNCH = SHARD == 3;
    constexpr bool COOP = SHARD == 4;

    extern __shared__ __align__(16) unsigned char smem[];
    const KpTables &tb = *p.tab;
    const int lane = threadIdx.x & 31, warp = threadIdx.x >> 5;
    const int rp = RP ? RP : tb.rp, nrounds = tb.nrounds, nhigh = tb.nhigh, nrows = tb.nrows;
    const uint32_t stride = RP ? (uint32_t)(NG * RP * 4) : tb.tile_stride, tk = tb.tile_kmers;
    const uint32_t rt_bytes = tb.rt_bytes;
    const int maxhs = tb.maxhs;

    double2 *logtab = (double2 *)smem;
    unsigned char *rt = smem + 2048;
    for (int i = threadIdx.x; i < 128; i += blockDim.x) logtab[i] = make_double2(kpc_logTab[2 * i], kpc_logTab[2 * i + 1]);
    for (uint32_t i = threadIdx.x; i < rt_bytes / 4; i += blockDim.x) ((uint32_t *)rt)[i] = ((const uint32_t *)p.rowtab)[i];
    __syncthreads();
    const uint16_t *round_start = (const uint16_t *)(rt + tb.rt_round_start);
    const uint8_t *row_level = rt + tb.rt_row_level;
    const uint16_t *xs_off = (const uint16_t *)(rt + tb.rt_xs_off);
    const uint32_t *xs = (const uint32_t *)(rt + tb.rt_xs);
    const uint16_t *bs_off = (const uint16_t *)(rt + tb.rt_bs_off);
    const uint16_t *bs = (const uint16_t *)(rt + tb.rt_bs);

    unsigned char *wm = smem + 2048 + rt_bytes + (size_t)(COOP ? 0 : warp) * tb.warp_smem_bytes[WIDE];
    float4 *S = (float4 *)wm;
    C *bc = (C *)(wm + (size_t)NG * rp * 16);
    uint32_t *hs1 = (uint32_t *)((unsigned char *)bc + (size_t)tk * 2 * sizeof(C));
    uint32_t *hs2 = hs1 + maxhs;
    int *s_nhs = (int *)(hs2 + maxhs);
    const double alpha = p.alpha, beta = p.beta, penalty = p.penalty;
    const KpFilterK fk = kp_filter_consts(alpha, beta, penalty);
    const float INF = __int_as_float(0x7f800000);
    const float *tbase = p.best;
    unsigned long long pol_first;
    asm("createpolicy.fractional.L2::evict_first.b64 %0, 1.0;" : "=l"(pol_first));

    for (;;) {
        uint32_t it = 0;
        if (COOP) {
            __syncthreads();
            if (threadIdx.x == 0) s_nhs[3] = (int)atomicAdd(p.counter, 1u);
            __syncthreads();
            it = (uint32_t)s_nhs[3];
        } else {
            if (lane == 0) it = atomicAdd(p.counter, 1u);
            it = __shfl_sync(0xffffffffu, it, 0);
        }
        if (it >= p.ntiles_wave) break;
        const uint32_t tile = p.tile_list[it];
        const int wave = ONE_LAUNCH ? (int)p.tile_wave[it] : 0;
        const bool leaf_tile = ONE_LAUNCH ? wave == 0 : (p.leaf_wave != 0);
        uint32_t ltile = tile;
        if (SHARDED) {
            const uint32_t dt = tile / p.view.hw_top;
            ltile = (uint32_t)p.view.slot[dt] * p.view.hw_top + (tile - dt * p.view.hw_top);
        }
        __syncwarp();
        if (!COOP || warp == 0) {
            int ns = 0, d = 0, e = 0;
            uint32_t m = 0, hw = 1;
            if (lane < nhigh) {
                e = tb.highpos[lane];
                hw = tb.highw[e];
                d = (int)((tile / hw) % tb.radix[e]);
                m = tb.digit_mask[e][d];
                ns = tb.ms_n[m];
            }
            int off = ns;
#pragma unroll
            for (int o = 1; o < 32; o <<= 1) {
                int x = __shfl_up_sync(0xffffffffu, off, o);
                if (lane >= o) off += x;
            }
            int total = __shfl_sync(0xffffffffu, off, 31);
            off -= ns;
            for (int j = 0; j < ns; j++) {
                int c1 = tb.mask_digit[e][tb.ms_c1[m][j]], c2 = tb.mask_digit[e][tb.ms_c2[m][j]];
                if (!SHARDED) {
                    hs1[off + j] = tile - (uint32_t)(d - c1) * hw;
                    hs2[off + j] = tile - (uint32_t)(d - c2) * hw;
                } else if (lane == nhigh - 1) {
                    const uint32_t rest = tile - (uint32_t)d * hw;
                    hs1[off + j] = ((uint32_t)p.view.slot[c1] * hw + rest) | ((uint32_t)p.view.owner[c1] << 28);
                    hs2[off + j] = ((uint32_t)p.view.slot[c2] * hw + rest) | ((uint32_t)p.view.owner[c2] << 28);
                } else {
                    hs1[off + j] = (ltile - (uint32_t)(d - c1) * hw) | ((uint32_t)p.my_rank << 28);
                    hs2[off + j] = (ltile - (uint32_t)(d - c2) * hw) | ((uint32_t)p.my_rank << 28);
                }
            }
            if (lane == 0) *s_nhs = total;
            if (KP_EXPERIMENTS && !SHARDED && !ONE_LAUNCH) {
                const int first = nhigh - p.evict_top;
                const int ptop_ = p.evict_top > 0 ? __shfl_sync(0xffffffffu, off, first > 0 ? first : 0) : 0x7fffffff;
                if (lane == 0) s_nhs[1] = ptop_;
                const int pfirst = nhigh - p.pf_top;
                const int pfs_ = (p.pf_top > 0 && pfirst > 0) ? __shfl_sync(0xffffffffu, off, pfirst) : 0;
                if (lane == 0) s_nhs[2] = pfs_;
            }
        }
        if (ONE_LAUNCH && wave > 0) {
            bool all_done = true;
            if (lane < 3 && wave - 1 - lane >= 0) {
                const int w = wave - 1 - lane;
                uint32_t c;
                asm volatile("ld.acquire.gpu.global.u32 %0, [%1];" : "=r"(c) : "l"(p.wave_done + w) : "memory");
                all_done = c == p.wave_size[w];
            }
            all_done = __all_sync(0xffffffffu, all_done);
            if (!all_done) {
                __syncwarp();
                const int n2 = 2 * *s_nhs;
                for (int j = lane; j < n2; j += 32) {
                    const uint32_t child = j & 1 ? hs2[j >> 1] : hs1[j >> 1];
                    unsigned spins = 0;
                    for (;;) {
                        uint32_t f;
                        asm volatile("ld.acquire.gpu.global.u8 %0, [%1];" : "=r"(f) : "l"(p.tile_done + child) : "memory");
                        if (f) break;
                        if (++spins > (1u << 22)) { atomicExch(p.err, 2); break; }
                        __nanosleep(200);
                    }
                }
            }
        }
        for (uint32_t kl = COOP ? threadIdx.x : lane; kl < tk; kl += COOP ? blockDim.x : 32) {
            size_t g = (size_t)tile * tk + kl;
            bc[kl * 2 + 0] = (C)(p.s0 ? p.e0[g] - p.s0[g] : p.e0[g]);
            bc[kl * 2 + 1] = (C)(p.s1 ? p.e1[g] - p.s1[g] : p.e1[g]);
        }
        __syncwarp();
        if (COOP) __syncthreads();
        const int nhs = *s_nhs;
        const int ptop = (KP_EXPERIMENTS && !SHARDED && !ONE_LAUNCH) ? s_nhs[1] : 0x7fffffff;
        const int pfs = (KP_EXPERIMENTS && !SHARDED && !ONE_LAUNCH) ? s_nhs[2] : 0;
        float4 *otile = (float4 *)(p.best + (size_t)ltile * stride);
        uint32_t pushm = 0;
        if (SHARD == 2) pushm = p.view.two_d ? p.view.push_mask2[tile / p.view.hw_second] : p.view.push_mask[tile / p.view.hw_top];

        {
            float v[NG * 4];
#pragma unroll
            for (int c = 0; c < NG * 4; c++) v[c] = INF;
            const int nchunk_all = (nrows + 31) >> 5;
            const int chunk0 = COOP ? warp : 0;
            const int nchunk = COOP ? (warp < nchunk_all ? 1 : 0) : nchunk_all;
            const int pend = COOP ? (nrows < 32 * (chunk0 + 1) ? nrows : 32 * (chunk0 + 1)) : nrows;
            const int nstep = nhs > 0 ? nchunk * nhs : 0;
            float4 xa0[NG], xb0[NG], xa1[NG], xb1[NG];
#if KP_PIPE_DEPTH == 3
            float4 xa2[NG], xb2[NG];
#endif
            const float4 *tb4 = (const float4 *)tbase;
            const uint32_t stride4 = stride >> 2;
            int ls = 0, lrow = lane + 32 * chunk0;
            const float4 *lptr = tb4 + (lrow < nrows ? lrow : nrows - 1);
            int lrowc = lrow < nrows ? lrow : nrows - 1;
            int us = 0, urow = lane + 32 * chunk0;
            int ps = 0, pchunk = 32 * chunk0;
            const uint32_t *pf_hs = (lane & 16) ? hs2 : hs1;
            const int pf_g = (lane >> 2) & 3, pf_line = (lane & 3) * 8;
            const float4 *pf_ptr = tb4 + pf_g * rp + pf_line;
            const bool pf_bulk = KP_EXPERIMENTS && p.pf_bulk != 0;
            const bool pf_on = (pf_bulk || pf_g < NG) && p.pf_dist >= 0;
#define KP_FL_PREFETCH()                                                                              \
    if (pchunk < pend) {                                                                              \
        if (KP_EXPERIMENTS && !SHARDED && pf_bulk) {    \
            if (pf_on && ps >= pfs) {                                                                 \
                const uint32_t nb_ = (uint32_t)(nrows - pchunk < 32 ? nrows - pchunk : 32) * 16u;     \
                const float4 *c1_ = tb4 + (size_t)hs1[ps] * stride4 + pchunk, *c2_ = tb4 + (size_t)hs2[ps] * stride4 + pchunk; \
                _Pragma("unroll") for (int g = 0; g < NG; g++) {                                      \
                    asm volatile("cp.async.bulk.prefetch.L2.global [%0], %1;" ::"l"(c1_ + g * rp), "r"(nb_)); \
                    asm volatile("cp.async.bulk.prefetch.L2.global [%0], %1;" ::"l"(c2_ + g * rp), "r"(nb_)); \
                }                                                                                     \
            }                                                                                         \
        } else {                                                                                      \
            const uint32_t ph_ = pf_hs[ps];                                                           \
            if (pf_on && ps >= pfs && pchunk + pf_line < nrows && (!SHARDED || (int)(ph_ >> 28) == p.my_rank)) \
                asm volatile("prefetch.global.L2 [%0];" ::"l"(pf_ptr + (size_t)(SHARDED ? (ph_ & 0x0fffffffu) : ph_) * stride4 + pchunk)); \
        }                                                                                             \
        if (++ps == nhs) { ps = 0; pchunk += 32; }                                                    \
    }
#define KP_FL_LOAD(xa, xb)                                                                            \
    {                                                                                                 \
        KP_FL_PREFETCH()                                                                              \
        const float4 *a_, *b_;                                                                        \
        if (!SHARDED) {                                                                               \
            a_ = lptr + (size_t)hs1[ls] * stride4;                                                    \
            b_ = lptr + (size_t)hs2[ls] * stride4;                                                    \
        } else {     \
            const uint32_t h1_ = hs1[ls], h2_ = hs2[ls];                                              \
            a_ = (const float4 *)p.view.best[h1_ >> 28] + lrowc + (size_t)(h1_ & 0x0fffffffu) * stride4; \
            b_ = (const float4 *)p.view.best[h2_ >> 28] + lrowc + (size_t)(h2_ & 0x0fffffffu) * stride4; \
        }                                                                                             \
        if (KP_EXPERIMENTS && !SHARDED && !ONE_LAUNCH && ls >= ptop) {    \
            _Pragma("unroll") for (int g = 0; g < NG; g++) {                                          \
                xa[g] = kp_ldg_policy(a_ + g * rp, pol_first);                                        \
                xb[g] = kp_ldg_policy(b_ + g * rp, pol_first);                                        \
            }                                                                                         \
        } else {                                                                                      \
            _Pragma("unroll") for (int g = 0; g < NG; g++) {    \
                xa[g] = ONE_LAUNCH ? __ldcg(a_ + g * rp) : __ldg(a_ + g * rp);                        \
                xb[g] = ONE_LAUNCH ? __ldcg(b_ + g * rp) : __ldg(b_ + g * rp);                        \
            }                                                                                         \
        }                                                                                             \
        if (++ls == nhs) {                                                                            \
            ls = 0; lrow += 32;                                                                       \
            lrowc = lrow < nrows ? lrow : nrows - 1;                                                  \
            lptr = tb4 + lrowc;                                                                       \
        }                                                                                             \
    }
#define KP_FL_USE(xa, xb)                                                                             \
    {                                                                                                 \
        _Pragma("unroll") for (int g = 0; g < NG; g++) {    \
            const float2 lo_ = __fadd2_rn(make_float2(xa[g].x, xa[g].y), make_float2(xb[g].x, xb[g].y)); \
            const float2 hi_ = __fadd2_rn(make_float2(xa[g].z, xa[g].w), make_float2(xb[g].z, xb[g].w)); \
            v[4 * g + 0] = fminf(v[4 * g + 0], lo_.x);                                                \
            v[4 * g + 1] = fminf(v[4 * g + 1], lo_.y);                                                \
            v[4 * g + 2] = fminf(v[4 * g + 2], hi_.x);                                                \
            v[4 * g + 3] = fminf(v[4 * g + 3], hi_.y);                                                \
        }                                                                                             \
        if (++us == nhs) {                 \
            if (urow < nrows) {                                                                       \
                _Pragma("unroll") for (int g = 0; g < NG; g++)                                        \
                    S[g * rp + urow] = make_float4(v[4 * g], v[4 * g + 1], v[4 * g + 2], v[4 * g + 3]); \
            }                                                                                         \
            _Pragma("unroll") for (int c = 0; c < NG * 4; c++) v[c] = INF;                            \
            us = 0; urow += 32;                                                                       \
        }                                                                                             \
    }
#if KP_PIPE_DEPTH == 3
            if (nstep > 0) {
                for (int i = 0; i < p.pf_dist; i++) KP_FL_PREFETCH()
                KP_FL_LOAD(xa0, xb0)
                if (nstep > 1) KP_FL_LOAD(xa1, xb1)
            }
            for (int t = 0; t < nstep; t += 3) {
                if (t + 2 < nstep) KP_FL_LOAD(xa2, xb2)
                KP_FL_USE(xa0, xb0)
                if (t + 3 < nstep) KP_FL_LOAD(xa0, xb0)
                if (t + 1 < nstep) KP_FL_USE(xa1, xb1)
                if (t + 4 < nstep) KP_FL_LOAD(xa1, xb1)
                if (t + 2 < nstep) KP_FL_USE(xa2, xb2)
            }
#else
            if (nstep > 0) {
                for (int i = 0; i < p.pf_dist; i++) KP_FL_PREFETCH()
                KP_FL_LOAD(xa0, xb0)
            }
            int t = 0;
            for (; t + 2 <= nstep; t += 2) {
                KP_FL_LOAD(xa1, xb1)
                KP_FL_USE(xa0, xb0)
                if (t + 2 < nstep) KP_FL_LOAD(xa0, xb0)
                KP_FL_USE(xa1, xb1)
            }
            if (t < nstep) KP_FL_USE(xa0, xb0)
#endif
#undef KP_FL_LOAD
#undef KP_FL_USE
#undef KP_FL_PREFETCH
            if (nhs <= 0)
                for (int srow = COOP ? (int)threadIdx.x : lane; srow < nrows; srow += COOP ? (int)blockDim.x : 32) {
#pragma unroll
                    for (int g = 0; g < NG; g++) S[g * rp + srow] = make_float4(INF, INF, INF, INF);
                }
            __syncwarp();
            if (COOP) __syncthreads();
        }

        for (int rnd = 0; rnd < (COOP && warp != 0 ? 0 : nrounds); rnd++) {
            const int srow = round_start[rnd] + lane;
            if (srow < round_start[rnd + 1]) {
                float v[NG * 4];
#pragma unroll
                for (int g = 0; g < NG; g++) {
                    float4 x = S[g * rp + srow];
                    v[4 * g] = x.x; v[4 * g + 1] = x.y; v[4 * g + 2] = x.z; v[4 * g + 3] = x.w;
                }
                {
                    int i = xs_off[srow];
                    const int iend = xs_off[srow + 1];
                    for (; i + 2 <= iend; i += 2) {
                        const uint32_t pr = xs[i], pq = xs[i + 1];
                        const float4 *a = S + (pr & 0xFFFFu), *b = S + (pr >> 16);
                        const float4 *c = S + (pq & 0xFFFFu), *e = S + (pq >> 16);
#pragma unroll
                        for (int g = 0; g < NG; g++) {
                            const float4 xa = a[g * rp], xb = b[g * rp], xc = c[g * rp], xe = e[g * rp];
                            const float2 l1 = __fadd2_rn(make_float2(xa.x, xa.y), make_float2(xb.x, xb.y));
                            const float2 h1 = __fadd2_rn(make_float2(xa.z, xa.w), make_float2(xb.z, xb.w));
                            const float2 l2 = __fadd2_rn(make_float2(xc.x, xc.y), make_float2(xe.x, xe.y));
                            const float2 h2 = __fadd2_rn(make_float2(xc.z, xc.w), make_float2(xe.z, xe.w));
                            v[4 * g + 0] = kp_min3(v[4 * g + 0], l1.x, l2.x);
                            v[4 * g + 1] = kp_min3(v[4 * g + 1], l1.y, l2.y);
                            v[4 * g + 2] = kp_min3(v[4 * g + 2], h1.x, h2.x);
                            v[4 * g + 3] = kp_min3(v[4 * g + 3], h1.y, h2.y);
                        }
                    }
                    if (i < iend) {
                        const uint32_t pr = xs[i];
                        const float4 *a = S + (pr & 0xFFFFu), *b = S + (pr >> 16);
#pragma unroll
                        for (int g = 0; g < NG; g++) {
                            const float4 xa = a[g * rp], xb = b[g * rp];
                            const float2 lo_ = __fadd2_rn(make_float2(xa.x, xa.y), make_float2(xb.x, xb.y));
                            const float2 hi_ = __fadd2_rn(make_float2(xa.z, xa.w), make_float2(xb.z, xb.w));
                            v[4 * g + 0] = fminf(v[4 * g + 0], lo_.x);
                            v[4 * g + 1] = fminf(v[4 * g + 1], lo_.y);
                            v[4 * g + 2] = fminf(v[4 * g + 2], hi_.x);
                            v[4 * g + 3] = fminf(v[4 * g + 3], hi_.y);
                        }
                    }
                }
                C m[NB], u[NB];
#pragma unroll
                for (int b = 0; b < NB; b++) { m[b] = 0; u[b] = 0; }
                for (int i = bs_off[srow]; i < bs_off[srow + 1]; i++) {
                    const C *q = bc + (size_t)bs[i] * NB * 2;
                    if (!WIDE && NB % 2 == 0) {
#pragma unroll
                        for (int b = 0; b < NB; b += 2) {
                            const uint4 x = *(const uint4 *)(q + b * 2);
                            m[b] += x.x; u[b] += x.y; m[b + 1] += x.z; u[b + 1] += x.w;
                        }
                    } else {
#pragma unroll
                        for (int b = 0; b < NB; b++) { m[b] += q[b * 2 + 0]; u[b] += q[b * 2 + 1]; }
                    }
                }
                const bool leafrow = leaf_tile && row_level[srow] == 0;
                uint32_t need = 0;
                {
                    float mf[NB], uf[NB];
#pragma unroll
                    for (int b = 0; b < NB; b++) { mf[b] = (float)m[b]; uf[b] = (float)u[b]; }
#pragma unroll
                    for (int h = 0; h < (R0 + 1) / 2; h++) {
                        float2 Mf = make_float2(0.f, 0.f), Uf = make_float2(0.f, 0.f);
#pragma unroll
                        for (int b = 0; b < NB; b++) {
                            if ((kp_bm_c<R0>(2 * h) >> b) & 1) { Mf.x += mf[b]; Uf.x += uf[b]; }
                            if (2 * h + 1 < R0 && ((kp_bm_c<R0>(2 * h + 1) >> b) & 1)) { Mf.y += mf[b]; Uf.y += uf[b]; }
                        }
                        const float2 lb = kp_score_lower_bound2(Mf, Uf, fk);
                        if (!(lb.x > v[2 * h])) need |= 1u << (2 * h);
                        if (2 * h + 1 < R0 && !(lb.y > v[2 * h + 1])) need |= 1u << (2 * h + 1);
                    }
                    if (leafrow) need |= (1u << NB) - 1u;
                }
                float sfx[NG * 4];
#pragma unroll
                for (int c = 0; c < NG * 4; c++) sfx[c] = 0.f;
                uint32_t rupm = 0;
                if (need) {
                    const KpLogK K = kp_logk_load();
                    uint32_t todo = need;
                    while (todo) {
                        const int d = __ffs(todo) - 1;
                        todo &= todo - 1;
                        const unsigned bm = kp_bm<R0>(d);
                        C M_ = 0, U_ = 0;
#pragma unroll
                        for (int b = 0; b < NB; b++)
                            if ((bm >> b) & 1u) { M_ += m[b]; U_ += u[b]; }
                        float sf;
                        bool ru;
                        const bool leafcell = leafrow && d < NB;
                        if (leafcell || !kp_self_score_fast<C>(M_, U_, alpha, beta, penalty, logtab, K, sf, ru)) {
                            const double s_ = leafcell ? kp_leaf_score_nl(M_, U_, alpha, beta, penalty, logtab)
                                                       : kp_self_score_exact_nl<C>(M_, U_, alpha, beta, penalty, logtab);
                            sf = __double2float_rn(s_);
                            ru = (double)sf > s_;
                        }
                        if (ru) rupm |= 1u << d;
                        ((float *)(S + (d >> 2) * rp + srow))[d & 3] = sf;
                    }
#pragma unroll
                    for (int g = 0; g < NG; g++) {
                        const float4 x = S[g * rp + srow];
                        sfx[4 * g] = x.x; sfx[4 * g + 1] = x.y; sfx[4 * g + 2] = x.z; sfx[4 * g + 3] = x.w;
                    }
                }
                uint32_t flag = 0;
#define KP_FIN(D)                                                                                     \
    if ((need >> (D)) & 1u) {                                                                         \
        const float sf_ = sfx[D];                                                                     \
        if (sf_ < v[D] || (sf_ == v[D] && ((rupm >> (D)) & 1u))) { v[D] = sf_; flag |= 1u << (D); }   \
    }
#define KP_SP(D, A, B) v[D] = fminf(v[D], __fadd_rn(v[A], v[B]));
#define KP_SP2(D, A, B, A2, B2) v[D] = kp_min3(v[D], __fadd_rn(v[A], v[B]), __fadd_rn(v[A2], v[B2]));
                if (R0 == 1) {
                    KP_FIN(0)
                } else if (R0 == 3) {
                    KP_FIN(0) KP_FIN(1)
                    KP_SP(2, 0, 1) KP_FIN(2)
                } else if (R0 == 7) {
                    KP_FIN(0) KP_FIN(1) KP_FIN(2)
                    KP_SP(3, 0, 1) KP_FIN(3)
                    KP_SP(4, 0, 2) KP_FIN(4)
                    KP_SP(5, 1, 2) KP_FIN(5)
                    KP_SP2(6, 0, 5, 1, 4) KP_SP(6, 2, 3) KP_FIN(6)
                } else {
                    KP_FIN(0) KP_FIN(1) KP_FIN(2) KP_FIN(3)
                    KP_SP(4, 0, 2) KP_FIN(4)
                    KP_SP(5, 1, 3) KP_FIN(5)
                    KP_SP(6, 2, 1) KP_FIN(6)
                    KP_SP(7, 0, 3) KP_FIN(7)
                    KP_SP(8, 2, 3) KP_FIN(8)
                    KP_SP(9, 0, 1) KP_FIN(9)
                    KP_SP2(10, 1, 8, 2, 5) KP_SP(10, 3, 6) KP_FIN(10)
                    KP_SP2(11, 0, 8, 2, 7) KP_SP(11, 3, 4) KP_FIN(11)
                    KP_SP2(12, 0, 5, 1, 7) KP_SP(12, 3, 9) KP_FIN(12)
                    KP_SP2(13, 0, 6, 1, 4) KP_SP(13, 2, 9) KP_FIN(13)
                    KP_SP2(14, 6, 7, 8, 9) KP_SP2(14, 4, 5, 0, 10)
                    KP_SP2(14, 1, 11, 2, 12) KP_SP(14, 3, 13) KP_FIN(14)
                }
#undef KP_FIN
#undef KP_SP
#undef KP_SP2
#pragma unroll
                for (int c = R0; c < NG * 4; c++) v[c] = 0.f;
#pragma unroll
                for (int g = 0; g < NG; g++) {
                    float4 o = make_float4(v[4 * g], v[4 * g + 1], v[4 * g + 2], v[4 * g + 3]);
                    S[g * rp + srow] = o;
                    __stcs(otile + g * rp + srow, o);
                }
                p.flags[(size_t)ltile * rp + srow] = (uint16_t)flag;
                if (SHARD == 2) {
                    for (uint32_t pm = pushm; pm; pm &= pm - 1) {
                        const int r = __ffs(pm) - 1;
                        float4 *rt_ = (float4 *)(const_cast<float *>(p.view.best[r]) + (size_t)tile * stride);
#pragma unroll
                        for (int g = 0; g < NG; g++)
                            rt_[g * rp + srow] = make_float4(v[4 * g], v[4 * g + 1], v[4 * g + 2], v[4 * g + 3]);
                        const_cast<uint16_t *>(p.view.flags[r])[(size_t)tile * rp + srow] = (uint16_t)flag;
                    }
                }
            }
            __syncwarp();
        }
        if (ONE_LAUNCH) {
            __threadfence();
            __syncwarp();
            if (lane == 0) {
                asm volatile("st.release.gpu.global.u8 [%0], %1;" ::"l"(p.tile_done + tile), "r"(1u) : "memory");
                atomicAdd(p.wave_done + wave, 1u);
            }
        }
    }
}

__global__ void kp_pack_kernel(const KpTables *tab, const uint8_t *gen_mask, int k, const unsigned long long *codes,
                               const long long *pos, const long long *neg, unsigned long long n, long long *kmerM,
                               long long *kmerU, int *err)
{
    const KpTables &tb = *tab;
    for (unsigned long long i = blockIdx.x * (unsigned long long)blockDim.x + threadIdx.x; i < n;
         i += (unsigned long long)gridDim.x * blockDim.x) {
        unsigned long long code = codes[i];
        unsigned long long kidx = 0;
        int e = 0;
        bool ok = true;
        for (int s = 0; s < k; s++) {
            unsigned m = (unsigned)((code >> (4 * s)) & 15u);
            unsigned g = gen_mask[s];
            if (m == 0 || (m & (m - 1)) || !(m & g)) { ok = false; break; }
            if (g & (g - 1)) {
                kidx += (unsigned long long)tb.mask_digit[e][m] * tb.kw[e];
                e++;
            }
        }
        if (!ok || (k < 16 && (code >> (4 * k)) != 0)) { atomicExch(err, 1); continue; }
        atomicAdd((unsigned long long *)&kmerM[kidx], (unsigned long long)pos[i]);
        atomicAdd((unsigned long long *)&kmerU[kidx], (unsigned long long)neg[i]);
    }
}

__global__ void kp_expand_base_kernel(const KpTables *tab, unsigned long long nkmer, const long long *kmerM,
                                      const long long *kmerU, long long *expM, long long *expU)
{
    const KpTables &tb = *tab;
    const uint32_t tk = tb.tile_kmers;
    for (unsigned long long x = blockIdx.x * (unsigned long long)blockDim.x + threadIdx.x; x < nkmer;
         x += (unsigned long long)gridDim.x * blockDim.x) {
        unsigned long long rest = x, tile = 0, kl = 0;
        for (int e = 0; e < tb.npos; e++) {
            unsigned long long b = rest % tb.nbase[e];
            rest /= tb.nbase[e];
            if (tb.is_low[e]) kl += b * tb.lkw[e];
            else tile += b * tb.highw[e];
        }
        expM[tile * tk + kl] = kmerM[x];
        expU[tile * tk + kl] = kmerU[x];
    }
}

__global__ void kp_expand_pass_kernel(const KpTables *tab, int hi, unsigned long long total, long long *expM, long long *expU)
{
    const KpTables &tb = *tab;
    __shared__ uint32_t s_n[KP_MAXPOS], s_w[KP_MAXPOS], s_add[KP_MAXPOS];
    __shared__ uint32_t s_src[16][4];
    __shared__ uint32_t s_nsrc[16];
    const int nhigh = tb.nhigh;
    const int e = tb.highpos[hi];
    const uint32_t tk = tb.tile_kmers;
    if (threadIdx.x < nhigh) {
        const int h = threadIdx.x, f = tb.highpos[h];
        const uint32_t nb = tb.nbase[f];
        s_n[h] = h < hi ? tb.radix[f] : (h == hi ? tb.radix[f] - nb : nb);
        s_add[h] = h == hi ? nb : 0;
        s_w[h] = tb.highw[f];
    }
    if (threadIdx.x < 16) {
        const int d = threadIdx.x;
        int n = 0;
        if (d < tb.radix[e]) {
            const uint32_t m = tb.digit_mask[e][d];
            for (int b = 0; b < 4; b++)
                if ((m >> b) & 1u) s_src[d][n++] = (uint32_t)(d - tb.mask_digit[e][1u << b]) * tb.highw[e];
        }
        s_nsrc[d] = (uint32_t)n;
    }
    __syncthreads();
    for (unsigned long long x = blockIdx.x * (unsigned long long)blockDim.x + threadIdx.x; x < total;
         x += (unsigned long long)gridDim.x * blockDim.x) {
        uint32_t kl, tile = 0, d = 0;
        if (total <= 0xFFFFFFFFull) {
            const uint32_t x32 = (uint32_t)x;
            kl = x32 % tk;
            uint32_t r = x32 / tk;
            for (int h = 0; h < nhigh; h++) {
                const uint32_t n = s_n[h];
                const uint32_t dig = r % n + s_add[h];
                r /= n;
                if (h == hi) d = dig;
                tile += dig * s_w[h];
            }
        } else {
            kl = (uint32_t)(x % tk);
            unsigned long long r = x / tk;
            for (int h = 0; h < nhigh; h++) {
                const uint32_t n = s_n[h];
                const uint32_t dig = (uint32_t)(r % n) + s_add[h];
                r /= n;
                if (h == hi) d = dig;
                tile += dig * s_w[h];
            }
        }
        long long am = 0, au = 0;
        const uint32_t ns = s_nsrc[d];
        for (uint32_t i = 0; i < ns; i++) {
            const size_t src = (size_t)(tile - s_src[d][i]) * tk + kl;
            am += expM[src];
            au += expU[src];
        }
        const size_t dst = (size_t)tile * tk + kl;
        expM[dst] = am;
        expU[dst] = au;
    }
}

struct KpLoc { unsigned long long tile; uint32_t srow, d0; };

__device__ __forceinline__ KpLoc kp_locate_dev(const KpTables &tb, const uint16_t *srow_of_row, unsigned long long pat)
{
    KpLoc L;
    L.tile = 0; L.d0 = 0;
    uint32_t row = 0;
    for (int e = 0; e < tb.npos; e++) {
        uint32_t dig = (uint32_t)((pat / tb.extw[e]) % tb.radix[e]);
        if (e == tb.estar) L.d0 = dig;
        else if (tb.is_low[e]) row += dig * tb.roww[e];
        else L.tile += (unsigned long long)dig * tb.highw[e];
    }
    L.srow = srow_of_row[row];
    return L;
}

__device__ __forceinline__ float kp_view_best(const KpTables &tb, const KpView &vw, unsigned long long tile, uint32_t srow, uint32_t d0)
{
    int r;
    unsigned long long lt;
    kp_view_tile(vw, tile, r, lt);
    return vw.best[r][lt * tb.tile_stride + ((size_t)(d0 >> 2) * tb.rp + srow) * 4 + (d0 & 3)];
}

__device__ __forceinline__ bool kp_view_kept(const KpTables &tb, const KpView &vw, unsigned long long tile, uint32_t srow, uint32_t d0)
{
    int r;
    unsigned long long lt;
    kp_view_tile(vw, tile, r, lt);
    return (vw.flags[r][lt * tb.rp + srow] >> d0) & 1u;
}

__device__ __forceinline__ float kp_best_at(const KpTables &tb, const uint16_t *srow_of_row, const KpView &vw,
                                            unsigned long long pat)
{
    KpLoc L = kp_locate_dev(tb, srow_of_row, pat);
    return kp_view_best(tb, vw, L.tile, L.srow, L.d0);
}

__device__ __forceinline__ void kp_counts_from_expanded(const KpTables &tb, const uint8_t *rowtab, const long long *eM,
                                                        const long long *eU, unsigned long long tile, uint32_t srow,
                                                        uint32_t d0, unsigned long long &M, unsigned long long &U)
{
    const uint16_t *bs_off = (const uint16_t *)(rowtab + tb.rt_bs_off);
    const uint16_t *bs = (const uint16_t *)(rowtab + tb.rt_bs);
    const uint32_t nb = (uint32_t)tb.nb0;
    const unsigned bm = tb.r0 == 15 ? kpc_bm15[d0] : (tb.r0 == 7 ? kpc_bm7[d0] : (tb.r0 == 3 ? kpc_bm3[d0] : kpc_bm1[d0]));
    M = 0; U = 0;
    for (int i = bs_off[srow]; i < bs_off[srow + 1]; i++)
        for (uint32_t b = 0; b < nb; b++)
            if ((bm >> b) & 1u) {
                size_t g = (size_t)tile * tb.tile_kmers + (size_t)bs[i] * nb + b;
                M += (unsigned long long)eM[g];
                U += (unsigned long long)eU[g];
            }
}

__global__ void kp_cv_leaf_kernel(const KpTables *tab, const uint8_t *rowtab, const long long *eMtot, const long long *eUtot,
                                  const long long *eMte, const long long *eUte, double alpha, double beta, double penalty,
                                  const unsigned long long *pats, const unsigned long long *counts, unsigned long long cap,
                                  float *out)
{
    const KpTables &tb = *tab;
    const uint16_t *srow_of_row = (const uint16_t *)(rowtab + tb.rt_srow_of_row);
    const uint8_t *row_level = rowtab + tb.rt_row_level;
    __shared__ double2 logtab[128];
    for (int i = threadIdx.x; i < 128; i += blockDim.x) logtab[i] = make_double2(kpc_logTab[2 * i], kpc_logTab[2 * i + 1]);
    __syncthreads();
    unsigned long long n = counts[0] < cap ? counts[0] : cap;
    const KpLogK K = kp_logk_load();
    for (unsigned long long i = blockIdx.x * (unsigned long long)blockDim.x + threadIdx.x; i < n;
         i += (unsigned long long)gridDim.x * blockDim.x) {
        KpLoc L = kp_locate_dev(tb, srow_of_row, pats[i]);
        unsigned long long Mtr, Utr, Mte, Ute;
        kp_counts_from_expanded(tb, rowtab, eMtot, eUtot, L.tile, L.srow, L.d0, Mtr, Utr);
        kp_counts_from_expanded(tb, rowtab, eMte, eUte, L.tile, L.srow, L.d0, Mte, Ute);
        Mtr -= Mte;
        Utr -= Ute;
        bool kmer = row_level[L.srow] == 0 && L.d0 < (uint32_t)tb.nb0;
        unsigned long long x = L.tile;
        for (int h = 0; h < tb.nhigh; h++) {
            int e = tb.highpos[h];
            if (x % tb.radix[e] >= tb.nbase[e]) kmer = false;
            x /= tb.radix[e];
        }
        double t;
        if (kmer) {
            double s;
            kp_leaf_cv(Mtr, Utr, Mte, Ute, alpha, beta, penalty, logtab, s, t);
        } else {
            double lp, l1;
            kp_self_score_t<unsigned long long>(Mtr, Utr, alpha, beta, penalty, logtab, K, lp, l1);
            t = kp_test_ll_t<unsigned long long>(Mte, Ute, lp, l1);
        }
        out[i] = __double2float_rn(t);
    }
}

__device__ uint8_t kp_split_code_dev(const KpTables &tb, const uint16_t *srow_of_row, const KpView &vw,
                                     unsigned long long pat, unsigned long long *c1_out, unsigned long long *c2_out)
{
    KpLoc L = kp_locate_dev(tb, srow_of_row, pat);
    if (kp_view_kept(tb, vw, L.tile, L.srow, L.d0)) return 0xFF;
    float bv = __int_as_float(0x7f800000);
    uint8_t code = 0xFF;
    for (int e = 0; e < tb.npos; e++) {
        unsigned long long w = tb.extw[e];
        int d = (int)((pat / w) % tb.radix[e]);
        uint32_t m = tb.digit_mask[e][d];
        for (int j = 0; j < tb.ms_n[m]; j++) {
            int c1 = tb.mask_digit[e][tb.ms_c1[m][j]], c2 = tb.mask_digit[e][tb.ms_c2[m][j]];
            unsigned long long p1 = pat - (unsigned long long)(d - c1) * w, p2 = pat - (unsigned long long)(d - c2) * w;
            float v = __fadd_rn(kp_best_at(tb, srow_of_row, vw, p1), kp_best_at(tb, srow_of_row, vw, p2));
            if (v < bv) { bv = v; code = (uint8_t)(tb.pos_id[e] * 8 + j); *c1_out = p1; *c2_out = p2; }
        }
    }
    return code;
}

struct KpBtNode { unsigned long long pat, key; };

__device__ __forceinline__ void kp_backtrack_level(const KpTables &tb, const uint8_t *rowtab, const KpView &vw, int depth,
                                                   const KpBtNode *cur, KpBtNode *nxt, KpBtNode *leaves,
                                                   unsigned long long cap, unsigned long long *ctr, unsigned long long ncur)
{
    const uint16_t *srow_of_row = (const uint16_t *)(rowtab + tb.rt_srow_of_row);
    const int lane = threadIdx.x & 31;
    const unsigned long long nw = (unsigned long long)gridDim.x * (blockDim.x >> 5);
    for (unsigned long long i = (unsigned long long)blockIdx.x * (blockDim.x >> 5) + (threadIdx.x >> 5); i < ncur; i += nw) {
        KpBtNode nd;
        nd.pat = __ldcg(&cur[i].pat);
        nd.key = __ldcg(&cur[i].key);
        unsigned long long ntile = 0;
        uint32_t nrow = 0, nd0 = 0;
        for (int e = 0; e < tb.npos; e++) {
            uint32_t dig = (uint32_t)((nd.pat / tb.extw[e]) % tb.radix[e]);
            if (e == tb.estar) nd0 = dig;
            else if (tb.is_low[e]) nrow += dig * tb.roww[e];
            else ntile += (unsigned long long)dig * tb.highw[e];
        }
        KpLoc L;
        L.tile = ntile; L.d0 = nd0; L.srow = srow_of_row[nrow];
        bool kept = kp_view_kept(tb, vw, L.tile, L.srow, L.d0);
        auto child_best = [&](int e, int d, int c) -> float {
            unsigned long long ct = ntile;
            uint32_t cr = nrow, cd = nd0;
            if (e == tb.estar) cd = (uint32_t)c;
            else if (tb.is_low[e]) cr -= (uint32_t)(d - c) * tb.roww[e];
            else ct -= (unsigned long long)(d - c) * tb.highw[e];
            return kp_view_best(tb, vw, ct, srow_of_row[cr], cd);
        };
        float bv = __int_as_float(0x7f800000);
        int code = 0x7fffffff;
        unsigned long long b1 = 0, b2 = 0;
        if (!kept && lane < tb.npos) {
            const int e = lane;
            unsigned long long w = tb.extw[e];
            int d = (int)((nd.pat / w) % tb.radix[e]);
            uint32_t m = tb.digit_mask[e][d];
            const int ns = tb.ms_n[m];
            float v[7];
#pragma unroll
            for (int j = 0; j < 7; j++) {
                v[j] = __int_as_float(0x7f800000);
                if (j < ns) {
                    int c1 = tb.mask_digit[e][tb.ms_c1[m][j]], c2 = tb.mask_digit[e][tb.ms_c2[m][j]];
                    v[j] = __fadd_rn(child_best(e, d, c1), child_best(e, d, c2));
                }
            }
#pragma unroll
            for (int j = 0; j < 7; j++)
                if (j < ns && v[j] < bv) {
                    bv = v[j];
                    code = tb.pos_id[e] * 8 + j;
                    b1 = nd.pat - (unsigned long long)(d - (int)tb.mask_digit[e][tb.ms_c1[m][j]]) * w;
                    b2 = nd.pat - (unsigned long long)(d - (int)tb.mask_digit[e][tb.ms_c2[m][j]]) * w;
                }
        }
#pragma unroll
        for (int o = 16; o > 0; o >>= 1) {
            float ov = __shfl_down_sync(0xffffffffu, bv, o);
            int oc = __shfl_down_sync(0xffffffffu, code, o);
            unsigned long long o1 = __shfl_down_sync(0xffffffffu, b1, o), o2 = __shfl_down_sync(0xffffffffu, b2, o);
            if (ov < bv || (ov == bv && oc < code)) { bv = ov; code = oc; b1 = o1; b2 = o2; }
        }
        if (lane == 0) {
            if (kept || code == 0x7fffffff) {
                unsigned long long li = atomicAdd(&ctr[0], 1ULL);
                if (li < cap) leaves[li] = nd; else ctr[1] = 1;
            } else if (depth >= 63) {
                ctr[1] = 1;
            } else {
                unsigned long long ni = atomicAdd(&ctr[2 + depth + 1], 2ULL);
                if (ni + 2 > cap) ctr[1] = 1;
                else {
                    nxt[ni].pat = b1;
                    nxt[ni].key = nd.key;
                    nxt[ni + 1].pat = b2;
                    nxt[ni + 1].key = nd.key | (1ULL << (63 - depth));
                }
            }
        }
    }
}

__global__ void __launch_bounds__(256) kp_backtrack_level_kernel(const KpTables *tab, const uint8_t *rowtab, const KpView vw,
                                                                 int depth, const KpBtNode *cur, KpBtNode *nxt,
                                                                 KpBtNode *leaves, unsigned long long cap,
                                                                 unsigned long long *ctr)
{
    kp_backtrack_level(*tab, rowtab, vw, depth, cur, nxt, leaves, cap, ctr, ctr[2 + depth]);
}

__global__ void __launch_bounds__(256) kp_backtrack_all_kernel(const KpTables *tab, const uint8_t *rowtab, const KpView vw,
                                                               int levels, KpBtNode *fa, KpBtNode *fb, KpBtNode *leaves,
                                                               unsigned long long cap, unsigned long long *ctr)
{
    const KpTables &tb = *tab;
    for (int d = 0; d < levels; d++) {
        const unsigned long long ncur = __ldcg(&ctr[2 + d]);
        if (ncur == 0) break;
        kp_backtrack_level(tb, rowtab, vw, d, (d & 1) ? fb : fa, (d & 1) ? fa : fb, leaves, cap, ctr, ncur < cap ? ncur : cap);
        __threadfence();
        __syncthreads();
        if (threadIdx.x == 0) {
            atomicAdd(&ctr[72], 1ULL);
            const unsigned long long want = (unsigned long long)(d + 1) * gridDim.x;
            unsigned long long seen;
            do {
                asm volatile("ld.acquire.gpu.global.u64 %0, [%1];" : "=l"(seen) : "l"(ctr + 72) : "memory");
                if (seen < want) __nanosleep(100);
            } while (seen < want);
        }
        __syncthreads();
    }
}

__global__ void kp_backtrack_init_kernel(KpBtNode *fa, unsigned long long top, unsigned long long *ctr)
{
    if (threadIdx.x < 80) ctr[threadIdx.x] = 0;
    __syncthreads();
    if (threadIdx.x == 0) { fa[0].pat = top; fa[0].key = 0; ctr[2] = 1; }
}

__global__ void kp_backtrack_sort_kernel(const KpBtNode *leaves, const unsigned long long *counts,
                                         unsigned long long cap, unsigned long long *out, unsigned long long *keys_out)
{
    unsigned long long n = counts[0];
    if (n > cap) n = cap;
    __shared__ unsigned long long keys[256];
    for (unsigned long long i0 = (unsigned long long)blockIdx.x * blockDim.x; i0 < n; i0 += (unsigned long long)gridDim.x * blockDim.x) {
        unsigned long long i = i0 + threadIdx.x;
        unsigned long long mykey = i < n ? leaves[i].key : 0, rank = 0;
        for (unsigned long long base = 0; base < n; base += 256) {
            unsigned long long j = base + threadIdx.x;
            keys[threadIdx.x] = j < n ? leaves[j].key : ~0ULL;
            __syncthreads();
            unsigned long long lim = n - base < 256 ? n - base : 256;
            for (unsigned long long t = 0; t < lim; t++) rank += keys[t] < mykey;
            __syncthreads();
        }
        if (i < n) { out[rank] = leaves[i].pat; keys_out[rank] = mykey; }
    }
}

struct KpGreedyLeaf { unsigned long long pat, key; double loss, test; };

#define KP_GREEDY_ACC (KP_MAXPOS * 8 + 4)

__global__ void __launch_bounds__(256) kp_greedy_marginals_kernel(const KpTables *tab, const long long *kmerM, const long long *kmerU,
                                                                  const long long *testM, const long long *testU, int depth,
                                                                  const KpBtNode *cur, const unsigned long long *cur_size,
                                                                  const unsigned long long *ctr, unsigned long long big,
                                                                  unsigned long long *acc)
{
    const KpTables &tb = *tab;
    __shared__ unsigned long long marg[KP_GREEDY_ACC];
    __shared__ uint8_t s_bases[KP_MAXPOS][4];
    __shared__ uint32_t s_n[KP_MAXPOS];
    const unsigned long long ncur = ctr[2 + depth];
    const int npos = tb.npos;
    for (unsigned long long ni = 0; ni < ncur; ni++) {
        const unsigned long long total = cur_size[ni];
        const bool shared_node = total >= big;
        if (!shared_node && ni % gridDim.x != blockIdx.x) continue;
        const KpBtNode nd = cur[ni];
        __syncthreads();
        if (threadIdx.x < npos) {
            const int e = threadIdx.x;
            const unsigned m = tb.digit_mask[e][(int)((nd.pat / tb.extw[e]) % tb.radix[e])];
            int n = 0;
            for (int b = 0; b < 4; b++)
                if ((m >> b) & 1u) s_bases[e][n++] = (uint8_t)b;
            s_n[e] = (uint32_t)n;
        }
        for (int i = threadIdx.x; i < KP_GREEDY_ACC; i += blockDim.x) marg[i] = 0;
        __syncthreads();
        unsigned long long aM = 0, aU = 0, aTM = 0, aTU = 0;
        const unsigned long long first = shared_node ? (unsigned long long)blockIdx.x * blockDim.x + threadIdx.x : threadIdx.x;
        const unsigned long long step = shared_node ? (unsigned long long)gridDim.x * blockDim.x : blockDim.x;
        for (unsigned long long t = first; t < total; t += step) {
            unsigned long long r = t, kidx = 0;
            uint8_t pick[KP_MAXPOS];
            for (int e = 0; e < npos; e++) {
                const uint32_t n = s_n[e];
                const int b = s_bases[e][r % n];
                r /= n;
                pick[e] = (uint8_t)b;
                kidx += (unsigned long long)tb.mask_digit[e][1u << b] * tb.kw[e];
            }
            const unsigned long long M = (unsigned long long)kmerM[kidx], U = (unsigned long long)kmerU[kidx];
            aM += M; aU += U;
            if (testM) { aTM += (unsigned long long)testM[kidx]; aTU += (unsigned long long)testU[kidx]; }
            for (int e = 0; e < npos; e++)
                if (s_n[e] > 1) {
                    if (M) atomicAdd(&marg[(e * 4 + pick[e]) * 2 + 0], M);
                    if (U) atomicAdd(&marg[(e * 4 + pick[e]) * 2 + 1], U);
                }
        }
        if (aM) atomicAdd(&marg[KP_MAXPOS * 8 + 0], aM);
        if (aU) atomicAdd(&marg[KP_MAXPOS * 8 + 1], aU);
        if (aTM) atomicAdd(&marg[KP_MAXPOS * 8 + 2], aTM);
        if (aTU) atomicAdd(&marg[KP_MAXPOS * 8 + 3], aTU);
        __syncthreads();
        for (int i = threadIdx.x; i < KP_GREEDY_ACC; i += blockDim.x)
// ... 678 lines not shown
```

### kmerpapa_b200/csrc/kp_plan.cpp

```cpp
#include "kp_plan.h"

#include <string.h>

#include <algorithm>

namespace {

struct Letter {
    char ch;
    uint8_t mask;
    const char *bases;
    const char *digits;
    const char *splits;
};

const Letter kLetters[15] = {
    {'A', 1, "A", "A", ""},
    {'C', 2, "C", "C", ""},
    {'G', 4, "G", "G", ""},
    {'T', 8, "T", "T", ""},
    {'R', 5, "AG", "AGR", "AG"},
    {'Y', 10, "CT", "CTY", "CT"},
    {'S', 6, "GC", "GCS", "GC"},
    {'W', 9, "AT", "ATW", "AT"},
    {'K', 12, "GT", "GTK", "GT"},
    {'M', 3, "AC", "ACM", "AC"},
    {'B', 14, "CGT", "CGTSYKB", "CKGYTS"},
    {'D', 13, "AGT", "AGTRWKD", "AKGWTR"},
    {'H', 11, "ACT", "ACTMWYH", "AYCWTM"},
    {'V', 7, "ACG", "ACGMRSV", "ASCRGM"},
    {'N', 15, "ACGT", "ACGTRYSWKMBDHVN", "SWKMRYABCDGHTV"},
};

const Letter *find_letter(char c)
{
    for (const Letter &l : kLetters)
        if (l.ch == c) return &l;
    return nullptr;
}

int popc4(unsigned m) { return (m & 1) + ((m >> 1) & 1) + ((m >> 2) & 1) + ((m >> 3) & 1); }

const uint8_t kDigitBases3[3] = {1, 2, 3};
const uint8_t kDigitBases7[7] = {1, 2, 4, 3, 5, 6, 7};
const uint8_t kDigitBases15[15] = {1, 2, 4, 8, 5, 10, 6, 9, 12, 3, 14, 13, 11, 7, 15};

}

int kp_build_host_plan(const char *gen_pat, KpHostPlan &P, std::string &err, bool lattice)
{
    P.lattice = lattice;
    size_t len = strlen(gen_pat);
    if (len < 1 || len > KP_MAXK) { err = "general pattern length must be 1.." + std::to_string(KP_MAXK); return 1; }
    P.gen = gen_pat;
    P.k = (int)len;
    KpTables &t = P.t;
    memset(&t, 0, sizeof t);
    memset(t.mask_digit, 0xFF, sizeof t.mask_digit);

    for (const Letter &l : kLetters) {
        int ns = (int)strlen(l.splits) / 2;
        t.ms_n[l.mask] = (uint8_t)ns;
        for (int j = 0; j < ns; j++) {
            t.ms_c1[l.mask][j] = find_letter(l.splits[2 * j])->mask;
            t.ms_c2[l.mask][j] = find_letter(l.splits[2 * j + 1])->mask;
        }
    }

    int npos = 0;
    uint64_t npat = 1, nkmer = 1;
    int total_level = 0;
    for (int i = 0; i < P.k; i++) {
        const Letter *g = find_letter(gen_pat[i]);
        if (!g) { err = std::string("not an IUPAC letter: '") + gen_pat[i] + "'"; return 2; }
        P.gen_mask[i] = g->mask;
        P.eff_of_pos[i] = 0xFF;
        int radix = (int)strlen(g->digits);
        if (radix == 1) continue;
        if (npos >= KP_MAXPOS) { err = "too many multi-letter positions (max " + std::to_string(KP_MAXPOS) + ")"; return 3; }
        int e = npos++;
        P.eff_of_pos[i] = (uint8_t)e;
        t.pos_id[e] = (uint8_t)i;
        t.radix[e] = (uint8_t)radix;
        t.nbase[e] = (uint8_t)strlen(g->bases);
        t.extw[e] = npat;
        if (nkmer >= (1ull << 31)) { err = "too many k-mers"; return 5; }
        t.kw[e] = (uint32_t)nkmer;
        for (int d = 0; d < radix; d++) {
            uint8_t m = find_letter(g->digits[d])->mask;
            t.digit_mask[e][d] = m;
            t.mask_digit[e][m] = (uint8_t)d;
        }
        for (int b = 0; b < t.nbase[e]; b++)
            if (g->digits[b] != g->bases[b]) { err = "internal: base/digit order mismatch"; return 4; }
        const uint8_t *want = radix == 3 ? kDigitBases3 : radix == 7 ? kDigitBases7 : kDigitBases15;
        for (int d = 0; d < radix; d++) {
            unsigned got = 0;
            for (int b = 0; b < 4; b++)
                if ((t.digit_mask[e][d] >> b) & 1) got |= 1u << t.mask_digit[e][1 << b];
            if (got != want[d]) { err = "internal: digit structure mismatch"; return 4; }
        }
        if (npat > (UINT64_MAX / 16)) { err = "pattern table too large"; return 5; }
        npat *= (uint64_t)radix;
        nkmer *= (uint64_t)t.nbase[e];
        total_level += t.nbase[e] - 1;
    }
    P.npat = npat;
    P.nkmer = nkmer;
    t.npos = npos;
    t.total_level = (uint32_t)total_level;

    std::vector<int> byradix(npos);
    for (int e = 0; e < npos; e++) byradix[e] = e;
    std::stable_sort(byradix.begin(), byradix.end(), [&](int a, int b) { return t.radix[a] > t.radix[b]; });
    uint32_t cells = 1;
    for (int e : byradix)
        if ((uint64_t)cells * t.radix[e] <= KP_MAX_TILE) { t.is_low[e] = 1; cells *= t.radix[e]; }
    t.estar = npos > 0 ? byradix[0] : -1;
    t.r0 = npos > 0 ? t.radix[t.estar] : 1;
    t.nb0 = npos > 0 ? t.nbase[t.estar] : 1;
    t.ng = (t.r0 + 3) / 4;
    std::vector<int> rowpos;
    uint32_t roww = 1, lkw = (uint32_t)t.nb0, hw = 1, tk = (uint32_t)t.nb0;
    if (t.estar >= 0) t.lkw[t.estar] = 1;
    for (int e = 0; e < npos; e++) {
        if (t.is_low[e]) {
            t.nlow++;
            if (e == t.estar) continue;
            rowpos.push_back(e);
            t.roww[e] = roww;
            t.lkw[e] = lkw;
            roww *= t.radix[e];
            lkw *= t.nbase[e];
            tk *= t.nbase[e];
        } else {
            t.highpos[t.nhigh++] = (uint8_t)e;
            t.highw[e] = hw;
            if ((uint64_t)hw * t.radix[e] >= (1ull << 31)) {
                if (lattice) { err = "too many tiles"; return 6; }
                hw = 0;
            }
            hw *= t.radix[e];
        }
    }
    t.nrows = (int32_t)roww;
    t.rp = (t.nrows + 7) & ~7;
    t.tile_cells = cells;
    t.tile_stride = (uint32_t)(t.ng * t.rp * 4);
    t.tile_kmers = tk;
    t.ntiles = hw;
    const uint64_t ntiles = hw;

    const int nrows = t.nrows;
    std::vector<std::vector<std::pair<int, int>>> xsplit(nrows);
    std::vector<std::vector<uint8_t>> xrank(nrows);
    std::vector<std::vector<uint16_t>> bases(nrows);
    std::vector<int> level(nrows, 0);
    for (int r = 0; r < nrows; r++) {
        int dig[KP_MAXPOS] = {0};
        uint32_t x = (uint32_t)r;
        for (int e : rowpos) { dig[e] = (int)(x % t.radix[e]); x /= t.radix[e]; }
        std::vector<uint32_t> acc(1, 0);
        for (int e : rowpos) {
            uint8_t m = t.digit_mask[e][dig[e]];
            level[r] += popc4(m) - 1;
            for (int j = 0; j < t.ms_n[m]; j++) {
                int c1 = t.mask_digit[e][t.ms_c1[m][j]], c2 = t.mask_digit[e][t.ms_c2[m][j]];
                if (c1 == 0xFF || c2 == 0xFF || c1 >= dig[e] || c2 >= dig[e]) { err = "internal: split table"; return 7; }
                xsplit[r].push_back({r - (dig[e] - c1) * (int)t.roww[e], r - (dig[e] - c2) * (int)t.roww[e]});
                xrank[r].push_back((uint8_t)(t.pos_id[e] * 8 + j));
            }
            std::vector<uint32_t> nxt;
            for (uint32_t a : acc)
                for (int b = 0; b < 4; b++)
                    if ((m >> b) & 1) nxt.push_back(a + (uint32_t)t.mask_digit[e][1 << b] * (t.lkw[e] / (uint32_t)t.nb0));
            acc.swap(nxt);
        }
        std::sort(acc.begin(), acc.end());
        for (uint32_t a : acc) bases[r].push_back((uint16_t)a);
    }
    std::vector<int> height(nrows, 0), pending(nrows, 0);
    std::vector<std::vector<int>> parents(nrows);
    for (int r = 0; r < nrows; r++) {
        std::vector<int> ch;
        for (auto &pr : xsplit[r]) { ch.push_back(pr.first); ch.push_back(pr.second); }
        std::sort(ch.begin(), ch.end());
        ch.erase(std::unique(ch.begin(), ch.end()), ch.end());
        pending[r] = (int)ch.size();
        for (int c : ch) parents[c].push_back(r);
    }
    for (int r = nrows - 1; r >= 0; r--)
        for (int q : parents[r]) height[r] = std::max(height[r], height[q] + 1);
    std::vector<int> ready, order;
    std::vector<uint16_t> round_start(1, 0);
    for (int r = 0; r < nrows; r++)
        if (pending[r] == 0) ready.push_back(r);
    while ((int)order.size() < nrows) {
        if (ready.empty()) { err = "internal: row schedule"; return 8; }
        std::sort(ready.begin(), ready.end(), [&](int a, int b) {
            if (height[a] != height[b]) return height[a] > height[b];
            if (xsplit[a].size() != xsplit[b].size()) return xsplit[a].size() > xsplit[b].size();
            return a < b;
        });
        int take = std::min<int>(32, (int)ready.size());
        std::vector<int> now(ready.begin(), ready.begin() + take);
        ready.erase(ready.begin(), ready.begin() + take);
        std::sort(now.begin(), now.end(), [&](int a, int b) {
            if (xsplit[a].size() != xsplit[b].size()) return xsplit[a].size() < xsplit[b].size();
            return a < b;
        });
        for (int r : now) order.push_back(r);
        round_start.push_back((uint16_t)order.size());
        for (int r : now)
            for (int q : parents[r])
                if (--pending[q] == 0) ready.push_back(q);
    }
    t.nrounds = (int32_t)round_start.size() - 1;
    P.row_of_srow.assign(order.begin(), order.end());
    P.srow_of_row.assign(nrows, 0);
    for (int s = 0; s < nrows; s++) P.srow_of_row[order[s]] = (uint16_t)s;

    {
        std::vector<uint8_t> &B = P.rowtab;
        B.clear();
        auto align = [&](size_t a) { while (B.size() % a) B.push_back(0); };
        auto put16 = [&](uint32_t v) { B.push_back((uint8_t)(v & 0xFF)); B.push_back((uint8_t)((v >> 8) & 0xFF)); };
        auto put32 = [&](uint32_t v) { for (int i = 0; i < 4; i++) B.push_back((uint8_t)(v >> (8 * i))); };
        t.rt_round_start = (uint32_t)B.size();
        for (uint16_t v : round_start) put16(v);
        align(4);
        t.rt_row_level = (uint32_t)B.size();
        for (int s = 0; s < nrows; s++) B.push_back((uint8_t)level[order[s]]);
        align(4);
        t.rt_xs_off = (uint32_t)B.size();
        {
            uint32_t o = 0;
            for (int s = 0; s < nrows; s++) { put16(o); o += (uint32_t)xsplit[order[s]].size(); }
            put16(o);
            if (o > 65535) { err = "internal: split list too long"; return 8; }
        }
        align(4);
        t.rt_xs = (uint32_t)B.size();
        for (int s = 0; s < nrows; s++)
            for (auto &pr : xsplit[order[s]])
                put32((uint32_t)P.srow_of_row[pr.first] | ((uint32_t)P.srow_of_row[pr.second] << 16));
        align(4);
        t.rt_xs_rank = (uint32_t)B.size();
        for (int s = 0; s < nrows; s++)
            for (uint8_t rk : xrank[order[s]]) B.push_back(rk);
        align(4);
        t.rt_bs_off = (uint32_t)B.size();
        {
            uint32_t o = 0;
            for (int s = 0; s < nrows; s++) { put16(o); o += (uint32_t)bases[order[s]].size(); }
            put16(o);
            if (o > 65535) { err = "internal: base list too long"; return 8; }
        }
        align(4);
        t.rt_bs = (uint32_t)B.size();
        for (int s = 0; s < nrows; s++)
            for (uint16_t b : bases[order[s]]) put16(b);
        align(4);
        t.rt_srow_of_row = (uint32_t)B.size();
        for (int r = 0; r < nrows; r++) put16(P.srow_of_row[r]);
        align(16);
        t.rt_bytes = (uint32_t)B.size();
    }
    t.maxhs = (uint32_t)((7 * t.nhigh + 3) & ~3);
    if (t.maxhs < 4) t.maxhs = 4;
    for (int wide = 0; wide < 2; wide++) {
        size_t b = (size_t)t.ng * t.rp * 16;
        b += (size_t)tk * 2 * (wide ? 8 : 4);
        b += (size_t)t.maxhs * 8 + 16;
        t.warp_smem_bytes[wide] = (uint32_t)((b + 15) & ~(size_t)15);
    }

    memset(&P.ft, 0, sizeof P.ft);
    if (!lattice) {
        t.ntiles = 0;
        P.hl_off.assign(1, 0);
        return 0;
    }
    {
        KpFiberTables &f = P.ft;
        int fhi = -1;
        for (int i = 0; i < t.nhigh && fhi < 0; i++)
            if (t.radix[t.highpos[i]] == KP_FIBER_DIGITS) fhi = i;
        if (t.r0 == 15 && nrows == KP_FIBER_ROWS && t.rp == 232 && rowpos.size() == 2 && fhi >= 0) {
            f.ok = 1;
            f.fhi = fhi;
            f.fe = t.highpos[fhi];
            f.hw = t.highw[f.fe];
            f.nfibers = (uint32_t)(ntiles / KP_FIBER_DIGITS);
            std::vector<int> frow_srow(nrows);
            for (int s = 0; s < nrows; s++) frow_srow[s] = s;
            std::stable_sort(frow_srow.begin(), frow_srow.end(), [&](int a, int b) { return level[order[a]] < level[order[b]]; });
            std::vector<int> frow_of_srow(nrows);
            for (int fr = 0; fr < nrows; fr++) frow_of_srow[frow_srow[fr]] = fr;
            int maxlvl = 0;
            for (int r = 0; r < nrows; r++) maxlvl = std::max(maxlvl, level[r]);
            if (maxlvl != KP_FIBER_ROW_LEVELS - 1) { err = "internal: fiber row levels"; return 9; }
            for (int l = 0; l <= KP_FIBER_ROW_LEVELS; l++) f.lvl_start[l] = 0;
            for (int r = 0; r < nrows; r++) f.lvl_start[level[r] + 1]++;
            for (int l = 0; l < KP_FIBER_ROW_LEVELS; l++) f.lvl_start[l + 1] += f.lvl_start[l];
            std::vector<uint8_t> &B = P.fibertab;
            B.clear();
            auto align = [&](size_t a) { while (B.size() % a) B.push_back(0); };
            auto put16 = [&](uint32_t v) { B.push_back((uint8_t)(v & 0xFF)); B.push_back((uint8_t)((v >> 8) & 0xFF)); };
            f.ft_srow_of_frow = (uint32_t)B.size();
            for (int fr = 0; fr < nrows; fr++) B.push_back((uint8_t)frow_srow[fr]);
            align(4);
            f.ft_frow_of_srow = (uint32_t)B.size();
            for (int s = 0; s < t.rp; s++) B.push_back(s < nrows ? (uint8_t)frow_of_srow[s] : (uint8_t)0xFF);
            align(4);
            f.ft_xs_off = (uint32_t)B.size();
            {
                uint32_t o = 0;
                for (int fr = 0; fr < nrows; fr++) { put16(o); o += (uint32_t)xsplit[order[frow_srow[fr]]].size(); }
                put16(o);
            }
            align(4);
            f.ft_xs = (uint32_t)B.size();
            for (int fr = 0; fr < nrows; fr++)
                for (auto &pr : xsplit[order[frow_srow[fr]]]) {
                    const int c1 = frow_of_srow[P.srow_of_row[pr.first]], c2 = frow_of_srow[P.srow_of_row[pr.second]];
                    if (c1 >= fr || c2 >= fr) { err = "internal: fiber row order"; return 9; }
                    put16((uint32_t)c1 | ((uint32_t)c2 << 8));
                }
            align(4);
            f.ft_bs_off = (uint32_t)B.size();
            {
                uint32_t o = 0;
                for (int fr = 0; fr < nrows; fr++) { put16(o); o += (uint32_t)bases[order[frow_srow[fr]]].size(); }
                put16(o);
            }
            align(4);
            f.ft_bs = (uint32_t)B.size();
            for (int fr = 0; fr < nrows; fr++)
                for (uint16_t b : bases[order[frow_srow[fr]]]) B.push_back((uint8_t)b);
            align(16);
            f.ft_bytes = (uint32_t)B.size();
            f.maxhs = (uint32_t)((7 * (t.nhigh - 1) + 3) & ~3);
            if (f.maxhs < 4) f.maxhs = 4;
        }
    }
    int nhl = 1;
    for (int i = 0; i < t.nhigh; i++) nhl += t.nbase[t.highpos[i]] - 1;
    std::vector<uint8_t> tl(ntiles);
    P.hl_off.assign((size_t)nhl + 1, 0);
    for (uint64_t tile = 0; tile < ntiles; tile++) {
        uint64_t x = tile;
        int l = 0;
        for (int i = 0; i < t.nhigh; i++) {
            int e = t.highpos[i];
            l += popc4(t.digit_mask[e][x % t.radix[e]]) - 1;
            x /= t.radix[e];
        }
        tl[tile] = (uint8_t)l;
        P.hl_off[(size_t)l + 1]++;
    }
    for (int l = 0; l < nhl; l++) P.hl_off[(size_t)l + 1] += P.hl_off[(size_t)l];
    P.tile_order.resize(ntiles);
    {
        std::vector<uint64_t> cur(P.hl_off.begin(), P.hl_off.end() - 1);
        for (uint64_t tile = 0; tile < ntiles; tile++) P.tile_order[cur[tl[tile]]++] = (uint32_t)tile;
    }
    if (P.ft.ok) {
        const KpFiberTables &f = P.ft;
        const int nfl = nhl - 3;
        std::vector<uint64_t> cnt((size_t)nfl + 1, 0);
        for (uint64_t tile = 0; tile < ntiles; tile++)
            if ((tile / f.hw) % KP_FIBER_DIGITS == 0) cnt[(size_t)tl[tile] + 1]++;
        for (int l = 0; l < nfl; l++) cnt[(size_t)l + 1] += cnt[(size_t)l];
        P.fl_off = cnt;
        P.fiber_order.resize(cnt[(size_t)nfl]);
        std::vector<uint64_t> cur(cnt.begin(), cnt.end() - 1);
        for (uint64_t tile = 0; tile < ntiles; tile++)
            if ((tile / f.hw) % KP_FIBER_DIGITS == 0) P.fiber_order[cur[tl[tile]]++] = (uint32_t)tile;
        if (P.fiber_order.size() != f.nfibers) { err = "internal: fiber count"; return 9; }
    }
    return 0;
}

void kp_locate(const KpHostPlan &P, uint64_t pat, uint64_t *tile, uint32_t *srow, uint32_t *d0)
{
    const KpTables &t = P.t;
    uint64_t tl = 0;
    uint32_t row = 0, d = 0;
    for (int e = 0; e < t.npos; e++) {
        uint32_t dig = (uint32_t)((pat / t.extw[e]) % t.radix[e]);
        if (e == t.estar) d = dig;
        else if (t.is_low[e]) row += dig * t.roww[e];
        else tl += (uint64_t)dig * t.highw[e];
    }
    *tile = tl;
    *srow = P.srow_of_row[row];
    *d0 = d;
}

void kp_num2masks(const KpHostPlan &P, uint64_t num, uint8_t *masks_out)
{
    for (int i = 0; i < P.k; i++) {
        uint8_t e = P.eff_of_pos[i];
        if (e == 0xFF) { masks_out[i] = P.gen_mask[i]; continue; }
        masks_out[i] = P.t.digit_mask[e][num % P.t.radix[e]];
        num /= P.t.radix[e];
    }
}
```

### kmerpapa_b200/csrc/kp_tables.h

```cpp
#pragma once
#include <stdint.h>

#define KP_MAXK 32
#define KP_MAXPOS 16
#define KP_MAX_TILE 4096
#define KP_MAXHS (KP_MAXPOS * 7)

struct KpTables {
    int32_t npos;
    int32_t nlow, nhigh;
    int32_t estar;
    int32_t r0, nb0, ng;
    int32_t nrows, rp;
    int32_t nrounds;
    uint32_t tile_cells, tile_stride, tile_kmers;
    uint32_t ntiles;
    uint32_t total_level;

    uint8_t pos_id[KP_MAXPOS];
    uint8_t radix[KP_MAXPOS];
    uint8_t nbase[KP_MAXPOS];
    uint8_t is_low[KP_MAXPOS];
    uint8_t highpos[KP_MAXPOS];
    uint32_t roww[KP_MAXPOS];
    uint32_t highw[KP_MAXPOS];
    uint32_t kw[KP_MAXPOS];
    uint32_t lkw[KP_MAXPOS];
    uint64_t extw[KP_MAXPOS];

    uint8_t digit_mask[KP_MAXPOS][16];
    uint8_t mask_digit[KP_MAXPOS][16];
    uint8_t ms_n[16];
    uint8_t ms_c1[16][7];
    uint8_t ms_c2[16][7];

    uint32_t rt_bytes;
    uint32_t rt_round_start;
    uint32_t rt_row_level;
    uint32_t rt_xs_off;
    uint32_t rt_xs;
    uint32_t rt_xs_rank;
    uint32_t rt_bs_off;
    uint32_t rt_bs;
    uint32_t rt_srow_of_row;
    uint32_t maxhs;
    uint32_t warp_smem_bytes[2];
};

#define KP_FIBER_ROWS 225
#define KP_FIBER_DIGITS 15
#define KP_FIBER_ROW_LEVELS 7
struct KpFiberTables {
    int32_t ok;
    int32_t fe;
    int32_t fhi;
    uint32_t hw;
    uint32_t nfibers;
    uint32_t lvl_start[KP_FIBER_ROW_LEVELS + 1];
    uint32_t ft_bytes;
    uint32_t ft_srow_of_frow;
    uint32_t ft_frow_of_srow;
    uint32_t ft_xs_off;
    uint32_t ft_xs;
    uint32_t ft_bs_off;
    uint32_t ft_bs;
    uint32_t maxhs;
};
```

Before: 93.94 billion.

## Pack global tile table densely as row-major cells instead of padded digit groups

Changes the global best-score tile layout from digit-group-major with padded rows (NG*rp*4 floats) to a dense row-major layout of nrows*r0 cells rounded to 32 floats. Loads in the DP kernels and the fiber kernel now stream contiguous float4 quads, cutting padded bytes from global traffic and simplifying prefetch addressing. Stores become a separate pass that transposes the shared-memory tile back to the dense layout, and the shared-memory pitch is padded by one row to reduce bank conflicts. This adds per-element division/modulo scatter into shared memory and an extra barrier and pass at tile output.

```diff
diff --git a/kmerpapa_b200/csrc/kp_api.cu b/kmerpapa_b200/csrc/kp_api.cu
--- a/kmerpapa_b200/csrc/kp_api.cu
+++ b/kmerpapa_b200/csrc/kp_api.cu
@@ -79,7 +79,6 @@
     bool one_launch = false;
 };
 
-#define KP_RP_NN 232
 #ifndef KP_FIBER_DEFAULT
 #define KP_FIBER_DEFAULT false
 #endif
@@ -295,7 +294,7 @@
     uint64_t tile; uint32_t srow, d0;
     kp_locate(p->host, patnum, &tile, &srow, &d0);
     const KpTables &t = p->host.t;
-    if (table_elem) *table_elem = tile * t.tile_stride + ((uint64_t)(d0 >> 2) * t.rp + srow) * 4 + (d0 & 3);
+    if (table_elem) *table_elem = kp_table_elem(t, tile, srow, d0);
     if (kept_elem) *kept_elem = tile * (uint64_t)t.rp + srow;
     if (kept_bit) *kept_bit = d0;
     return 0;
@@ -437,7 +436,7 @@
         prm.counter = p->d_counters + l;
         prm.leaf_wave = (l == 0);
         uint64_t ntile = hi - lo;
-        const int nchunk = (t.nrows + 31) / 32;
+        const int nchunk = (int)((((uint32_t)t.nrows * 15u + 3u) / 4u + 127u) / 128u);
         if (p->coop_tail && t.r0 == 15 && ntile <= (uint64_t)p->sm_count && nchunk <= KP_MAX_WARPS) {
             const size_t smc = 2048 + t.rt_bytes + (size_t)t.warp_smem_bytes[wide];
             if (t.rp == KP_RP_NN) launch_dp_r0<15, KP_RP_NN, 4>(wide, (int)ntile, nchunk * 32, smc, st, prm);
@@ -613,7 +612,7 @@
             return rc;
         uint64_t tile; uint32_t srow, d0;
         kp_locate(p->host, p->host.npat - 1, &tile, &srow, &d0);
-        size_t top = (size_t)tile * t.tile_stride + ((size_t)(d0 >> 2) * t.rp + srow) * 4 + (d0 & 3);
+        const size_t top = kp_table_elem(t, tile, srow, d0);
         KP_CUDA(cudaMemcpyAsync(h_top, d_train + top, sizeof(float), cudaMemcpyDeviceToHost, st));
         KP_CUDA(cudaStreamSynchronize(st));
     }
@@ -643,7 +642,7 @@
     unsigned char *h = (unsigned char *)h_stage;
     uint64_t tile; uint32_t srow, d0;
     kp_locate(p->host, p->host.npat - 1, &tile, &srow, &d0);
-    const size_t top = (size_t)tile * t.tile_stride + ((size_t)(d0 >> 2) * t.rp + srow) * 4 + (d0 & 3);
+    const size_t top = kp_table_elem(t, tile, srow, d0);
     KP_CUDA(cudaMemcpyAsync(h, ctr, 16, cudaMemcpyDeviceToHost, st));
     KP_CUDA(cudaMemcpyAsync(h + 16, d_train + top, sizeof(float), cudaMemcpyDeviceToHost, st));
     KP_CUDA(cudaMemcpyAsync(h + 32, keys, cap * 8, cudaMemcpyDeviceToHost, st));
diff --git a/kmerpapa_b200/csrc/kp_fiber.cuh b/kmerpapa_b200/csrc/kp_fiber.cuh
--- a/kmerpapa_b200/csrc/kp_fiber.cuh
+++ b/kmerpapa_b200/csrc/kp_fiber.cuh
@@ -58,6 +58,11 @@
         P2[idx] = make_float4(v[8], v[9], v[10], v[11]);
         Q0[idx] = v[12]; Q1[idx] = v[13]; Q2[idx] = v[14];
     }
+    __device__ __forceinline__ float *cell(int idx, int d) const
+    {
+        float *b = (float *)P0;
+        return d < 12 ? b + ((d >> 2) * KP_FIBER_CELLS + idx) * 4 + (d & 3) : b + d * KP_FIBER_CELLS + idx;
+    }
 };
 
 __device__ __forceinline__ void kp_fiber_split1(const KpFiberS &S, int ia, int ib, float *v)
@@ -102,9 +107,10 @@
 __global__ void __launch_bounds__(KP_FIBER_THREADS, 1) kp_dp_fiber_kernel(const KpFiberParams p)
 {
     typedef typename KpCnt<WIDE>::type C;
-    constexpr int R0 = 15, NB = 4, NT = KP_FIBER_THREADS, NR = KP_FIBER_ROWS, RP = 232;
-    constexpr int TILE4 = 4 * RP;
-    constexpr int NJ = KP_FIBER_DIGITS * TILE4;
+    constexpr int R0 = 15, NB = 4, NT = KP_FIBER_THREADS, NR = KP_FIBER_ROWS, RP = KP_RP_NN;
+    constexpr int TILE4 = KP_NN_STRIDE / 4;
+    constexpr int NQ = (NR * R0 + 3) / 4;
+    constexpr int NJ = KP_FIBER_DIGITS * NQ;
 
     extern __shared__ __align__(16) unsigned char smem[];
     const KpTables &tb = *p.tab;
@@ -200,12 +206,10 @@
 
         for (int j0 = tid; j0 < ((p.dbg & 1) ? 0 : NJ); j0 += 2 * NT) {
             const int j1 = j0 + NT;
-            const int x0 = j0 / TILE4, r0 = j0 - x0 * TILE4;
-            const int x1 = j1 / TILE4, r1 = j1 - x1 * TILE4;
-            const int g0 = r0 / RP, srow0 = r0 - g0 * RP;
-            const int g1 = r1 / RP, srow1 = r1 - g1 * RP;
-            const bool ok0 = srow0 < NR, ok1 = j1 < NJ && srow1 < NR;
-            const size_t o0 = (size_t)x0 * hwf * TILE4 + r0, o1 = (size_t)x1 * hwf * TILE4 + r1;
+            const int x0 = j0 / NQ, q0 = j0 - x0 * NQ;
+            const int x1 = j1 / NQ, q1 = j1 - x1 * NQ;
+            const bool ok1 = j1 < NJ;
+            const size_t o0 = (size_t)x0 * hwf * TILE4 + q0, o1 = (size_t)x1 * hwf * TILE4 + q1;
             float4 acc0 = make_float4(INF, INF, INF, INF), acc1 = acc0;
             for (int s0 = 0; s0 < nhs; s0 += 4) {
                 float4 a0[4], b0[4], a1[4], b1[4];
@@ -214,7 +218,7 @@
                     a0[q] = b0[q] = a1[q] = b1[q] = make_float4(INF, INF, INF, INF);
                     if (s0 + q < nhs) {
                         const float4 *c1 = tb4 + (size_t)hs1[s0 + q] * TILE4, *c2 = tb4 + (size_t)hs2[s0 + q] * TILE4;
-                        if (ok0) { a0[q] = __ldg(c1 + o0); b0[q] = __ldg(c2 + o0); }
+                        a0[q] = __ldg(c1 + o0); b0[q] = __ldg(c2 + o0);
                         if (ok1) { a1[q] = __ldg(c1 + o1); b1[q] = __ldg(c2 + o1); }
                     }
                 }
@@ -224,19 +228,12 @@
                     acc1 = kp_min4(acc1, a1[q], b1[q]);
                 }
             }
-            if (ok0) {
-                const int idx = x0 * NR + frow_of_srow[srow0];
-                if (g0 == 0) S.P0[idx] = acc0;
-                else if (g0 == 1) S.P1[idx] = acc0;
-                else if (g0 == 2) S.P2[idx] = acc0;
-                else { S.Q0[idx] = acc0.x; S.Q1[idx] = acc0.y; S.Q2[idx] = acc0.z; }
-            }
-            if (ok1) {
-                const int idx = x1 * NR + frow_of_srow[srow1];
-                if (g1 == 0) S.P0[idx] = acc1;
-                else if (g1 == 1) S.P1[idx] = acc1;
-                else if (g1 == 2) S.P2[idx] = acc1;
-                else { S.Q0[idx] = acc1.x; S.Q1[idx] = acc1.y; S.Q2[idx] = acc1.z; }
+            const float c0[4] = {acc0.x, acc0.y, acc0.z, acc0.w}, c1[4] = {acc1.x, acc1.y, acc1.z, acc1.w};
+#pragma unroll
+            for (int c = 0; c < 4; c++) {
+                const int f0 = 4 * q0 + c, f1 = 4 * q1 + c;
+                if (f0 < NR * R0) *S.cell(x0 * NR + frow_of_srow[f0 / R0], f0 % R0) = c0[c];
+                if (ok1 && f1 < NR * R0) *S.cell(x1 * NR + frow_of_srow[f1 / R0], f1 % R0) = c1[c];
             }
         }
         __syncthreads();
@@ -392,16 +389,14 @@
         }
 
         for (int j = tid; j < NJ; j += NT) {
-            const int x = j / TILE4, r = j - x * TILE4;
-            const int g = r / RP, srow = r - g * RP;
-            if (srow >= NR) continue;
-            const int idx = x * NR + frow_of_srow[srow];
-            float4 o;
-            if (g == 0) o = S.P0[idx];
-            else if (g == 1) o = S.P1[idx];
-            else if (g == 2) o = S.P2[idx];
-            else o = make_float4(S.Q0[idx], S.Q1[idx], S.Q2[idx], 0.f);
-            __stcs((float4 *)p.best + (size_t)(base + x * hwf) * TILE4 + r, o);
+            const int x = j / NQ, q = j - x * NQ;
+            float o[4];
+#pragma unroll
+            for (int c = 0; c < 4; c++) {
+                const int f = 4 * q + c;
+                o[c] = f < NR * R0 ? *S.cell(x * NR + frow_of_srow[f / R0], f % R0) : 0.f;
+            }
+            __stcs((float4 *)p.best + (size_t)(base + x * hwf) * TILE4 + q, make_float4(o[0], o[1], o[2], o[3]));
         }
         for (int j = tid; j < KP_FIBER_DIGITS * RP; j += NT) {
             const int x = j / RP, srow = j - x * RP;
diff --git a/kmerpapa_b200/csrc/kp_kernels.cuh b/kmerpapa_b200/csrc/kp_kernels.cuh
--- a/kmerpapa_b200/csrc/kp_kernels.cuh
+++ b/kmerpapa_b200/csrc/kp_kernels.cuh
@@ -284,8 +284,12 @@
     extern __shared__ __align__(16) unsigned char smem[];
     const KpTables &tb = *p.tab;
     const int lane = threadIdx.x & 31, warp = threadIdx.x >> 5;
-    const int rp = RP ? RP : tb.rp, nrounds = tb.nrounds, nhigh = tb.nhigh, nrows = tb.nrows;
-    const uint32_t stride = RP ? (uint32_t)(NG * RP * 4) : tb.tile_stride, tk = tb.tile_kmers;
+    static_assert(RP == 0 || (R0 == 15 && RP == KP_RP_NN), "a compile-time pitch is the all-N tile shape's");
+    const int rp = RP ? RP : tb.rp, nrounds = tb.nrounds, nhigh = tb.nhigh, nrows = RP ? KP_NN_ROWS : tb.nrows;
+    const int sp = kp_smem_pitch(rp);
+    const uint32_t stride = RP ? (uint32_t)KP_NN_STRIDE : tb.tile_stride, tk = tb.tile_kmers;
+    constexpr int CH4 = NG * 32;
+    const int ncell = nrows * R0, nq = (ncell + 3) >> 2;
     const uint32_t rt_bytes = tb.rt_bytes;
     const int maxhs = tb.maxhs;
 
@@ -303,7 +307,7 @@
 
     unsigned char *wm = smem + 2048 + rt_bytes + (size_t)(COOP ? 0 : warp) * tb.warp_smem_bytes[WIDE];
     float4 *S = (float4 *)wm;
-    C *bc = (C *)(wm + (size_t)NG * rp * 16);
+    C *bc = (C *)(wm + (size_t)NG * sp * 16);
     uint32_t *hs1 = (uint32_t *)((unsigned char *)bc + (size_t)tk * 2 * sizeof(C));
     uint32_t *hs2 = hs1 + maxhs;
     int *s_nhs = (int *)(hs2 + maxhs);
@@ -420,73 +424,73 @@
             float v[NG * 4];
 #pragma unroll
             for (int c = 0; c < NG * 4; c++) v[c] = INF;
-            const int nchunk_all = (nrows + 31) >> 5;
+            const int nchunk_all = (nq + CH4 - 1) / CH4;
             const int chunk0 = COOP ? warp : 0;
             const int nchunk = COOP ? (warp < nchunk_all ? 1 : 0) : nchunk_all;
-            const int pend = COOP ? (nrows < 32 * (chunk0 + 1) ? nrows : 32 * (chunk0 + 1)) : nrows;
+            const int pend = COOP ? (nq < CH4 * (chunk0 + 1) ? nq : CH4 * (chunk0 + 1)) : nq;
             const int nstep = nhs > 0 ? nchunk * nhs : 0;
+            const float4 zero4 = make_float4(0.f, 0.f, 0.f, 0.f);
             float4 xa0[NG], xb0[NG], xa1[NG], xb1[NG];
+#pragma unroll
+            for (int g = 0; g < NG; g++) xa0[g] = xb0[g] = xa1[g] = xb1[g] = zero4;
 #if KP_PIPE_DEPTH == 3
             float4 xa2[NG], xb2[NG];
+#pragma unroll
+            for (int g = 0; g < NG; g++) xa2[g] = xb2[g] = zero4;
 #endif
             const float4 *tb4 = (const float4 *)tbase;
             const uint32_t stride4 = stride >> 2;
-            int ls = 0, lrow = lane + 32 * chunk0;
-            const float4 *lptr = tb4 + (lrow < nrows ? lrow : nrows - 1);
-            int lrowc = lrow < nrows ? lrow : nrows - 1;
-            int us = 0, urow = lane + 32 * chunk0;
-            int ps = 0, pchunk = 32 * chunk0;
+            int ls = 0, lq = lane + CH4 * chunk0;
+            int us = 0, uq = lane + CH4 * chunk0;
+            int ps = 0, pchunk = CH4 * chunk0;
             const uint32_t *pf_hs = (lane & 16) ? hs2 : hs1;
-            const int pf_g = (lane >> 2) & 3, pf_line = (lane & 3) * 8;
-            const float4 *pf_ptr = tb4 + pf_g * rp + pf_line;
+            const int pf_line = (lane & 15) * 8;
+            const float4 *pf_ptr = tb4 + pf_line;
             const bool pf_bulk = KP_EXPERIMENTS && p.pf_bulk != 0;
-            const bool pf_on = (pf_bulk || pf_g < NG) && p.pf_dist >= 0;
+            const bool pf_on = (pf_bulk || pf_line < CH4) && p.pf_dist >= 0;
 #define KP_FL_PREFETCH()                                                                              \
     if (pchunk < pend) {                                                                              \
         if (KP_EXPERIMENTS && !SHARDED && pf_bulk) {    \
             if (pf_on && ps >= pfs) {                                                                 \
-                const uint32_t nb_ = (uint32_t)(nrows - pchunk < 32 ? nrows - pchunk : 32) * 16u;     \
+                const uint32_t nb_ = (uint32_t)(pend - pchunk < CH4 ? pend - pchunk : CH4) * 16u;     \
                 const float4 *c1_ = tb4 + (size_t)hs1[ps] * stride4 + pchunk, *c2_ = tb4 + (size_t)hs2[ps] * stride4 + pchunk; \
-                _Pragma("unroll") for (int g = 0; g < NG; g++) {                                      \
-                    asm volatile("cp.async.bulk.prefetch.L2.global [%0], %1;" ::"l"(c1_ + g * rp), "r"(nb_)); \
-                    asm volatile("cp.async.bulk.prefetch.L2.global [%0], %1;" ::"l"(c2_ + g * rp), "r"(nb_)); \
-                }                                                                                     \
+                asm volatile("cp.async.bulk.prefetch.L2.global [%0], %1;" ::"l"(c1_), "r"(nb_));      \
+                asm volatile("cp.async.bulk.prefetch.L2.global [%0], %1;" ::"l"(c2_), "r"(nb_));      \
             }                                                                                         \
         } else {                                                                                      \
             const uint32_t ph_ = pf_hs[ps];                                                           \
-            if (pf_on && ps >= pfs && pchunk + pf_line < nrows && (!SHARDED || (int)(ph_ >> 28) == p.my_rank)) \
+            if (pf_on && ps >= pfs && pchunk + pf_line < pend && (!SHARDED || (int)(ph_ >> 28) == p.my_rank)) \
                 asm volatile("prefetch.global.L2 [%0];" ::"l"(pf_ptr + (size_t)(SHARDED ? (ph_ & 0x0fffffffu) : ph_) * stride4 + pchunk)); \
         }                                                                                             \
-        if (++ps == nhs) { ps = 0; pchunk += 32; }                                                    \
+        if (++ps == nhs) { ps = 0; pchunk += CH4; }                                                   \
     }
 #define KP_FL_LOAD(xa, xb)                                                                            \
     {                                                                                                 \
         KP_FL_PREFETCH()                                                                              \
         const float4 *a_, *b_;                                                                        \
         if (!SHARDED) {                                                                               \
-            a_ = lptr + (size_t)hs1[ls] * stride4;                                                    \
-            b_ = lptr + (size_t)hs2[ls] * stride4;                                                    \
+            a_ = tb4 + lq + (size_t)hs1[ls] * stride4;                                                \
+            b_ = tb4 + lq + (size_t)hs2[ls] * stride4;                                                \
         } else {     \
             const uint32_t h1_ = hs1[ls], h2_ = hs2[ls];                                              \
-            a_ = (const float4 *)p.view.best[h1_ >> 28] + lrowc + (size_t)(h1_ & 0x0fffffffu) * stride4; \
-            b_ = (const float4 *)p.view.best[h2_ >> 28] + lrowc + (size_t)(h2_ & 0x0fffffffu) * stride4; \
+            a_ = (const float4 *)p.view.best[h1_ >> 28] + lq + (size_t)(h1_ & 0x0fffffffu) * stride4; \
+            b_ = (const float4 *)p.view.best[h2_ >> 28] + lq + (size_t)(h2_ & 0x0fffffffu) * stride4; \
         }                                                                                             \
+        const int lim_ = pend - lq;    \
         if (KP_EXPERIMENTS && !SHARDED && !ONE_LAUNCH && ls >= ptop) {    \
-            _Pragma("unroll") for (int g = 0; g < NG; g++) {                                          \
-                xa[g] = kp_ldg_policy(a_ + g * rp, pol_first);                                        \
-                xb[g] = kp_ldg_policy(b_ + g * rp, pol_first);                                        \
-            }                                                                                         \
+            _Pragma("unroll") for (int g = 0; g < NG; g++)                                            \
+                if (g * 32 < lim_) {                                                                  \
+                    xa[g] = kp_ldg_policy(a_ + g * 32, pol_first);                                    \
+                    xb[g] = kp_ldg_policy(b_ + g * 32, pol_first);                                    \
+                }                                                                                     \
         } else {                                                                                      \
-            _Pragma("unroll") for (int g = 0; g < NG; g++) {    \
-                xa[g] = ONE_LAUNCH ? __ldcg(a_ + g * rp) : __ldg(a_ + g * rp);                        \
-                xb[g] = ONE_LAUNCH ? __ldcg(b_ + g * rp) : __ldg(b_ + g * rp);                        \
-            }                                                                                         \
+            _Pragma("unroll") for (int g = 0; g < NG; g++)    \
+                if (g * 32 < lim_) {                                                                  \
+                    xa[g] = ONE_LAUNCH ? __ldcg(a_ + g * 32) : __ldg(a_ + g * 32);                    \
+                    xb[g] = ONE_LAUNCH ? __ldcg(b_ + g * 32) : __ldg(b_ + g * 32);                    \
+                }                                                                                     \
         }                                                                                             \
-        if (++ls == nhs) {                                                                            \
-            ls = 0; lrow += 32;                                                                       \
-            lrowc = lrow < nrows ? lrow : nrows - 1;                                                  \
-            lptr = tb4 + lrowc;                                                                       \
-        }                                                                                             \
+        if (++ls == nhs) { ls = 0; lq += CH4; }                                                       \
     }
 #define KP_FL_USE(xa, xb)                                                                             \
     {                                                                                                 \
@@ -498,13 +502,16 @@
             v[4 * g + 2] = fminf(v[4 * g + 2], hi_.x);                                                \
             v[4 * g + 3] = fminf(v[4 * g + 3], hi_.y);                                                \
         }                                                                                             \
-        if (++us == nhs) {                 \
-            if (urow < nrows) {                                                                       \
-                _Pragma("unroll") for (int g = 0; g < NG; g++)                                        \
-                    S[g * rp + urow] = make_float4(v[4 * g], v[4 * g + 1], v[4 * g + 2], v[4 * g + 3]); \
+        if (++us == nhs) {    \
+            _Pragma("unroll") for (int c = 0; c < NG * 4; c++) {                                      \
+                const int f_ = 4 * (uq + (c >> 2) * 32) + (c & 3);     \
+                if (f_ < ncell) {                                                                     \
+                    const int sr_ = f_ / R0, d_ = f_ - sr_ * R0;                                      \
+                    ((float *)(S + (d_ >> 2) * sp + sr_))[d_ & 3] = v[c];                             \
+                }                                                                                     \
             }                                                                                         \
             _Pragma("unroll") for (int c = 0; c < NG * 4; c++) v[c] = INF;                            \
-            us = 0; urow += 32;                                                                       \
+            us = 0; uq += CH4;                                                                        \
         }                                                                                             \
     }
 #if KP_PIPE_DEPTH == 3
@@ -541,7 +548,7 @@
             if (nhs <= 0)
                 for (int srow = COOP ? (int)threadIdx.x : lane; srow < nrows; srow += COOP ? (int)blockDim.x : 32) {
 #pragma unroll
-                    for (int g = 0; g < NG; g++) S[g * rp + srow] = make_float4(INF, INF, INF, INF);
+                    for (int g = 0; g < NG; g++) S[g * sp + srow] = make_float4(INF, INF, INF, INF);
                 }
             __syncwarp();
             if (COOP) __syncthreads();
@@ -553,7 +560,7 @@
                 float v[NG * 4];
 #pragma unroll
                 for (int g = 0; g < NG; g++) {
-                    float4 x = S[g * rp + srow];
+                    float4 x = S[g * sp + srow];
                     v[4 * g] = x.x; v[4 * g + 1] = x.y; v[4 * g + 2] = x.z; v[4 * g + 3] = x.w;
                 }
                 {
@@ -565,7 +572,7 @@
                         const float4 *c = S + (pq & 0xFFFFu), *e = S + (pq >> 16);
 #pragma unroll
                         for (int g = 0; g < NG; g++) {
-                            const float4 xa = a[g * rp], xb = b[g * rp], xc = c[g * rp], xe = e[g * rp];
+                            const float4 xa = a[g * sp], xb = b[g * sp], xc = c[g * sp], xe = e[g * sp];
                             const float2 l1 = __fadd2_rn(make_float2(xa.x, xa.y), make_float2(xb.x, xb.y));
                             const float2 h1 = __fadd2_rn(make_float2(xa.z, xa.w), make_float2(xb.z, xb.w));
                             const float2 l2 = __fadd2_rn(make_float2(xc.x, xc.y), make_float2(xe.x, xe.y));
@@ -581,7 +588,7 @@
                         const float4 *a = S + (pr & 0xFFFFu), *b = S + (pr >> 16);
 #pragma unroll
                         for (int g = 0; g < NG; g++) {
-                            const float4 xa = a[g * rp], xb = b[g * rp];
+                            const float4 xa = a[g * sp], xb = b[g * sp];
                             const float2 lo_ = __fadd2_rn(make_float2(xa.x, xa.y), make_float2(xb.x, xb.y));
                             const float2 hi_ = __fadd2_rn(make_float2(xa.z, xa.w), make_float2(xb.z, xb.w));
                             v[4 * g + 0] = fminf(v[4 * g + 0], lo_.x);
@@ -652,11 +659,11 @@
                             ru = (double)sf > s_;
                         }
                         if (ru) rupm |= 1u << d;
-                        ((float *)(S + (d >> 2) * rp + srow))[d & 3] = sf;
+                        ((float *)(S + (d >> 2) * sp + srow))[d & 3] = sf;
                     }
 #pragma unroll
                     for (int g = 0; g < NG; g++) {
-                        const float4 x = S[g * rp + srow];
+                        const float4 x = S[g * sp + srow];
                         sfx[4 * g] = x.x; sfx[4 * g + 1] = x.y; sfx[4 * g + 2] = x.z; sfx[4 * g + 3] = x.w;
                     }
                 }
@@ -700,24 +707,30 @@
 #pragma unroll
                 for (int c = R0; c < NG * 4; c++) v[c] = 0.f;
 #pragma unroll
-                for (int g = 0; g < NG; g++) {
-                    float4 o = make_float4(v[4 * g], v[4 * g + 1], v[4 * g + 2], v[4 * g + 3]);
-                    S[g * rp + srow] = o;
-                    __stcs(otile + g * rp + srow, o);
-                }
+                for (int g = 0; g < NG; g++) S[g * sp + srow] = make_float4(v[4 * g], v[4 * g + 1], v[4 * g + 2], v[4 * g + 3]);
                 p.flags[(size_t)ltile * rp + srow] = (uint16_t)flag;
                 if (SHARD == 2) {
                     for (uint32_t pm = pushm; pm; pm &= pm - 1) {
                         const int r = __ffs(pm) - 1;
-                        float4 *rt_ = (float4 *)(const_cast<float *>(p.view.best[r]) + (size_t)tile * stride);
-#pragma unroll
-                        for (int g = 0; g < NG; g++)
-                            rt_[g * rp + srow] = make_float4(v[4 * g], v[4 * g + 1], v[4 * g + 2], v[4 * g + 3]);
                         const_cast<uint16_t *>(p.view.flags[r])[(size_t)tile * rp + srow] = (uint16_t)flag;
                     }
                 }
             }
             __syncwarp();
+        }
+        if (COOP) __syncthreads();
+        for (int q = COOP ? (int)threadIdx.x : lane; q < nq; q += COOP ? (int)blockDim.x : 32) {
+            float o[4];
+#pragma unroll
+            for (int c = 0; c < 4; c++) {
+                const int f = 4 * q + c, sr = f / R0, d = f - sr * R0;
+                o[c] = f < ncell ? ((const float *)(S + (d >> 2) * sp + sr))[d & 3] : 0.f;
+            }
+            const float4 o4 = make_float4(o[0], o[1], o[2], o[3]);
+            __stcs(otile + q, o4);
+            if (SHARD == 2)
+                for (uint32_t pm = pushm; pm; pm &= pm - 1)
+                    ((float4 *)(const_cast<float *>(p.view.best[__ffs(pm) - 1]) + (size_t)tile * stride))[q] = o4;
         }
         if (ONE_LAUNCH) {
             __threadfence();
@@ -862,7 +875,7 @@
     int r;
     unsigned long long lt;
     kp_view_tile(vw, tile, r, lt);
-    return vw.best[r][lt * tb.tile_stride + ((size_t)(d0 >> 2) * tb.rp + srow) * 4 + (d0 & 3)];
+    return vw.best[r][kp_table_elem(tb, lt, srow, d0)];
 }
 
 __device__ __forceinline__ bool kp_view_kept(const KpTables &tb, const KpView &vw, unsigned long long tile, uint32_t srow, uint32_t d0)
diff --git a/kmerpapa_b200/csrc/kp_plan.cpp b/kmerpapa_b200/csrc/kp_plan.cpp
--- a/kmerpapa_b200/csrc/kp_plan.cpp
+++ b/kmerpapa_b200/csrc/kp_plan.cpp
@@ -146,7 +146,11 @@
     t.nrows = (int32_t)roww;
     t.rp = (t.nrows + 7) & ~7;
     t.tile_cells = cells;
-    t.tile_stride = (uint32_t)(t.ng * t.rp * 4);
+    t.tile_stride = kp_dense_stride((uint32_t)t.nrows, (uint32_t)t.r0);
+    if (t.r0 == 15 && t.rp == KP_RP_NN && (t.nrows != KP_NN_ROWS || t.tile_stride != KP_NN_STRIDE)) {
+        err = "internal: all-N tile shape";
+        return 4;
+    }
     t.tile_kmers = tk;
     t.ntiles = hw;
     const uint64_t ntiles = hw;
@@ -269,7 +273,7 @@
     t.maxhs = (uint32_t)((7 * t.nhigh + 3) & ~3);
     if (t.maxhs < 4) t.maxhs = 4;
     for (int wide = 0; wide < 2; wide++) {
-        size_t b = (size_t)t.ng * t.rp * 16;
+        size_t b = (size_t)t.ng * kp_smem_pitch(t.rp) * 16;
         b += (size_t)tk * 2 * (wide ? 8 : 4);
         b += (size_t)t.maxhs * 8 + 16;
         t.warp_smem_bytes[wide] = (uint32_t)((b + 15) & ~(size_t)15);
diff --git a/kmerpapa_b200/csrc/kp_tables.h b/kmerpapa_b200/csrc/kp_tables.h
--- a/kmerpapa_b200/csrc/kp_tables.h
+++ b/kmerpapa_b200/csrc/kp_tables.h
@@ -5,6 +5,19 @@
 #define KP_MAXPOS 16
 #define KP_MAX_TILE 4096
 #define KP_MAXHS (KP_MAXPOS * 7)
+
+#define KP_NN_ROWS 225
+#define KP_RP_NN 232
+#define KP_NN_STRIDE 3392
+
+#ifdef __CUDACC__
+#define KP_HD __host__ __device__
+#else
+#define KP_HD
+#endif
+
+static inline KP_HD uint32_t kp_dense_stride(uint32_t nrows, uint32_t r0) { return (nrows * r0 + 31u) & ~31u; }
+static inline KP_HD int kp_smem_pitch(int rp) { return rp + 1; }
 
 struct KpTables {
     int32_t npos;
@@ -47,6 +60,11 @@
     uint32_t warp_smem_bytes[2];
 };
 
+static inline KP_HD uint64_t kp_table_elem(const KpTables &t, uint64_t tile, uint32_t srow, uint32_t d0)
+{
+    return tile * t.tile_stride + (uint64_t)srow * (uint32_t)t.r0 + d0;
+}
+
 #define KP_FIBER_ROWS 225
 #define KP_FIBER_DIGITS 15
 #define KP_FIBER_ROW_LEVELS 7
```

Result: slower. 91.32 billion, median of 6 (-2.8%).
